# sinamalakouti/CDDMSL

Hardware: AMD Instinct MI355X
Metric: images/sec (train step) VOC+Clipart RN50-C4 (higher is better)
Workload: dtype bf16

## Files before the change

cddmsl_amd/csrc/gemm_conv.hip:

```cpp
#include "common.h"
#include <cstdlib>
#include <type_traits>

namespace {

constexpr int BM = 128, BN = 128, KCH = 8;

struct FastDiv {
  unsigned mul, shr, d;
};
static inline FastDiv make_fastdiv(unsigned d) {
  FastDiv f;
  f.d = d;
  unsigned s = 0;
  while ((1ull << s) < d) ++s;
  f.shr = s;
  f.mul = (unsigned)(((1ull << 32) * ((1ull << s) - d)) / d + 1);
  return f;
}
__device__ __forceinline__ unsigned fdiv(unsigned n, const FastDiv& f) { return (__umulhi(n, f.mul) + n) >> f.shr; }

template <typename T> __device__ __forceinline__ float affine(float v, float sc, float bi) {
  return sizeof(T) <= 2 ? __builtin_fmaf(v, sc, bi) : v * sc + bi;
}
// ... 467 lines not shown
      }
  }

  stage(0);
  for (int kt = 0; kt < nkt; ++kt) {
    const int cur = kt & 1;
    if (kt + 1 < nkt) {
      stage(cur ^ 1);
      asm volatile("s_waitcnt vmcnt(8)" ::: "memory");
    } else {
      asm volatile("s_waitcnt vmcnt(0)" ::: "memory");
    }
    __builtin_amdgcn_s_barrier();
    u32x4 fa[2][2], fb[2][2];
#pragma unroll
    for (int i = 0; i < 2; ++i) {
      fa[0][i] = lds[cur][0][swz(wm * 64 + i * 32 + r, h)];
      fb[0][i] = lds[cur][1][swz(wn * 64 + i * 32 + r, h)];
    }
#pragma unroll
    for (int ks = 0; ks < KCH / 2; ++ks) {
      if (ks + 1 < KCH / 2) {
#pragma unroll
        for (int i = 0; i < 2; ++i) {
          fa[(ks + 1) & 1][i] = lds[cur][0][swz(wm * 64 + i * 32 + r, 2 * (ks + 1) + h)];
          fb[(ks + 1) & 1][i] = lds[cur][1][swz(wn * 64 + i * 32 + r, 2 * (ks + 1) + h)];
        }
      }
#pragma unroll
      for (int a = 0; a < 2; ++a)
#pragma unroll
        for (int b = 0; b < 2; ++b) Mma<T>::step(acc[a][b], fa[ks & 1][a], fb[ks & 1][b]);
    }
    asm volatile("s_waitcnt lgkmcnt(0)" ::: "memory");
    __builtin_amdgcn_s_barrier();
  }

  if (vec_ok) {
    float* ep = (float*)&lds[0][0][0] + wv * 2048;
    const int cg = lane & 7, rr = lane >> 3;
    const int n = n0 + wn * 64 + cg * 8;
    float sc[8], bi[8];
#pragma unroll
    for (int j = 0; j < 8; ++j) {
      sc[j] = (p.scale && n + j < p.Cout) ? p.scale[n + j] : 1.f;
      bi[j] = (p.bias && n + j < p.Cout) ? p.bias[n + j] : 0.f;
    }
#pragma unroll
    for (int a = 0; a < 2; ++a) {
      __syncthreads();
#pragma unroll
      for (int b = 0; b < 2; ++b)
#pragma unroll
        for (int g = 0; g < 16; ++g) {
          int row = (g & 3) + 8 * (g >> 2) + 4 * h, col = b * 32 + r;
          ep[row * 64 + ((((col >> 3) ^ (row & 7)) << 3) | (col & 7))] = acc[a][b][g];
        }
      __syncthreads();
      if (n < p.Cout) {
#pragma unroll
        for (int i = 0; i < 4; ++i) {
          int row = rr + 8 * i;
          int m = m0 + wm * 64 + a * 32 + row;
          if (m >= p.M) continue;
          const f32x4* src = (const f32x4*)(ep + row * 64 + ((cg ^ (row & 7)) << 3));
          f32x4 v0 = src[0], v1 = src[1];
          float v[8] = {v0[0], v0[1], v0[2], v0[3], v1[0], v1[1], v1[2], v1[3]};
#pragma unroll
          for (int j = 0; j < 8; ++j) v[j] = affine<T>(v[j], sc[j], bi[j]);
          if (p.residual) {
            float rv[8];
            if (rf32) load8<float>(p.residual + ((long)m * p.ldr + n) * 4, rv);
            else if (PRE) {
#pragma unroll
              for (int j = 0; j < 4; ++j) { rv[2 * j] = bf2f(rres[a][i][j] & 0xffff); rv[2 * j + 1] = bf2f(rres[a][i][j] >> 16); }
            } else if (p.res_pool) {
              const long po = pooled_row(p, m);
#pragma unroll
              for (int j = 0; j < 8; ++j) rv[j] = 0.f;
              if (po >= 0) load8<T>(p.residual + (po * p.ldr + n) * Mma<T>::ES, rv);
            } else load8<T>(p.residual + ((long)m * p.ldr + n) * Mma<T>::ES, rv);
            if (p.res_pool) {
#pragma unroll
              for (int j = 0; j < 8; ++j) rv[j] *= 0.25f;
            }
#pragma unroll
            for (int j = 0; j < 8; ++j) v[j] += rv[j];
          }
          if (p.relu) {
#pragma unroll
            for (int j = 0; j < 8; ++j) v[j] = fmaxf(v[j], 0.f);
          }
          if (p.relu_mask) {
            float mv[8];
            if (PRE) {
#pragma unroll
              for (int j = 0; j < 4; ++j) { mv[2 * j] = bf2f(rmsk[a][i][j] & 0xffff); mv[2 * j + 1] = bf2f(rmsk[a][i][j] >> 16); }
            } else load8<T>(p.relu_mask + ((long)m * p.ldm + n) * Mma<T>::ES, mv);
#pragma unroll
            for (int j = 0; j < 8; ++j) if (!(mv[j] > 0.f)) v[j] = 0.f;
          }
          if (p.out_f32 || Mma<T>::ES == 4) {
            f32x4* dst = (f32x4*)(p.y + ((long)m * p.ldy + n) * 4);
            f32x4 o0 = {v[0], v[1], v[2], v[3]}, o1 = {v[4], v[5], v[6], v[7]};
            dst[0] = o0; dst[1] = o1;
          } else {
            u32x4 o = {pack2bf(v[0], v[1]), pack2bf(v[2], v[3]), pack2bf(v[4], v[5]), pack2bf(v[6], v[7])};
            *(u32x4*)(p.y + ((long)m * p.ldy + n) * 2) = o;
          }
        }
      }
    }
    return;
  }
#pragma unroll
  for (int b = 0; b < 2; ++b) {
    int n = n0 + wn * 64 + b * 32 + r;
    if (n >= p.Cout) continue;
    float sc = p.scale ? p.scale[n] : 1.f;
    float bi = p.bias ? p.bias[n] : 0.f;
#pragma unroll
    for (int a = 0; a < 2; ++a) {
#pragma unroll
      for (int g = 0; g < 16; ++g) {
        int m = m0 + wm * 64 + a * 32 + (g & 3) + 8 * (g >> 2) + 4 * h;
        if (m >= p.M) continue;
        float v = affine<T>(acc[a][b][g], sc, bi);
        if (p.residual) v += Mma<T>::load(p.residual + ((long)m * p.ldr + n) * Mma<T>::ES);
        if (p.relu) v = fmaxf(v, 0.f);
        if (p.relu_mask && !(Mma<T>::load(p.relu_mask + ((long)m * p.ldm + n) * Mma<T>::ES) > 0.f)) v = 0.f;
        if (p.out_f32) *(float*)(p.y + ((long)m * p.ldy + n) * 4) = v;
        else Mma<T>::store(p.y + ((long)m * p.ldy + n) * Mma<T>::ES, v);
      }
    }
  }
}

struct WgradArgs {
  const char* x;
  const char* dy;
  float* dw;
  const float* scale;
  int Nimg, Hi, Wi, Cin, Ho, Wo, Cout, KH, KW, stride, pad, ldd, pool;
  int M, Kc, cpp, K, ncc;
  int mtiles_per_split;
  FastDiv dWo, dHo;
  int xrs;
  int ldo;
  int direct;
  long bx, bd, bo;
  const float* g0 = nullptr;
  const unsigned long long* mbits = nullptr;
  float* gpos = nullptr;
  float* ws = nullptr;
#ifdef CDDMSL_TILE_STAMPS
  unsigned long long* tstamps = nullptr;
#endif
};

constexpr int WM = 64;
constexpr int WROW = 16 + 4;

template <typename T> struct TrFrag;
template <> struct TrFrag<__bf16> {
  __device__ static __forceinline__ u32x4 read(const u32x4* base, int mrow0, int col0, int lane) {
    int g = lane >> 4, li = lane & 15, q = li >> 2, pp = li & 3;
    int hh = g >> 1;
    int col = col0 + 16 * (g & 1) + 4 * pp;
    const char* b = (const char*)base;
    const char* a0 = b + (long)(mrow0 + 8 * hh + q) * (WROW * 16) + col * 2;
    const char* a1 = a0 + 4 * (WROW * 16);
    i16x4 v0 = __builtin_amdgcn_ds_read_tr16_b64_v4i16((__attribute__((address_space(3))) i16x4*)a0);
    i16x4 v1 = __builtin_amdgcn_ds_read_tr16_b64_v4i16((__attribute__((address_space(3))) i16x4*)a1);
    u32x2 p0 = __builtin_bit_cast(u32x2, v0), p1 = __builtin_bit_cast(u32x2, v1);
    u32x4 r = {p0[0], p0[1], p1[0], p1[1]};
    return r;
  }
  static constexpr int MSTEP = 16;
};
template <> struct TrFrag<float> {
  __device__ static __forceinline__ u32x4 read(const u32x4* base, int mrow0, int col0, int lane) {
    int r = lane & 31, hh = lane >> 5;
    const char* b = (const char*)base;
    u32x4 v;
#pragma unroll
    for (int j = 0; j < 4; ++j) v[j] = *(const unsigned int*)(b + (long)(mrow0 + 4 * hh + j) * (WROW * 16) + (col0 + r) * 4);
    return v;
  }
  static constexpr int MSTEP = 8;
};

template <typename T>
__global__ __launch_bounds__(256, 2) void k_conv_wgrad(WgradArgs p) {
  constexpr int ES = Mma<T>::ES;
  constexpr int TC = 128 * ES / 16;
  constexpr int COLS = 256 / ES;
  __shared__ __attribute__((aligned(16))) u32x4 lds[2][WM * WROW];
  const int t = threadIdx.x, lane = t & 63, wv = t >> 6;
  const int ntn = (p.Cout + COLS - 1) / COLS, ntk = (p.K + COLS - 1) / COLS;
  int bid = xcd_remap(blockIdx.x, gridDim.x);
  const int tile_k = bid % ntk; bid /= ntk;
  const int tile_n = bid % ntn; bid /= ntn;
  const int split = bid;
  const int n0 = tile_n * COLS, k0 = tile_k * COLS;
  const int mt0 = split * p.mtiles_per_split;
  const int total_mt = (p.M + WM - 1) / WM;
  const int mt1 = min(mt0 + p.mtiles_per_split, total_mt);
  (void)TC;

  const int cc = t & 15, rb = t >> 4;
  const int kc = k0 * ES / 16 + cc;
  const bool vk = kc < p.Kc;
  const int pp = vk ? kc / p.cpp : 0, coff = vk ? kc - pp * p.cpp : 0;
  const int ky = pp / p.KW, kx = pp - ky * p.KW;
  const int nc = n0 * ES / 16 + cc;
  const bool vn = nc < p.ncc;
  const u32x4 zero = {0u, 0u, 0u, 0u};
  u32x4 rx[4], rd[4];

  auto gload = [&](int mt) {
#pragma unroll
    for (int i = 0; i < 4; ++i) {
      int m = mt * WM + rb + 16 * i;
      bool vmm = m < p.M;
      unsigned mm = vmm ? m : 0;
      unsigned tq = fdiv(mm, p.dWo);
      int ox = (int)(mm - tq * p.Wo);
      unsigned img = fdiv(tq, p.dHo);
      int oy = (int)(tq - img * p.Ho);
      if (!p.pool) {
        int iy = oy * p.stride - p.pad + ky, ix = ox * p.stride - p.pad + kx;
        bool ok = vmm && vk && iy >= 0 && iy < p.Hi && ix >= 0 && ix < p.Wi;
        rx[i] = ok ? *(const u32x4*)(p.x + ((((long)img * p.Hi + iy) * p.Wi + ix) * p.cpp + coff) * 16) : zero;
      } else {
        if (vmm && vk) {
          const char* b0 = p.x + ((((long)img * p.Hi + 2 * oy) * p.Wi + 2 * ox) * p.cpp + coff) * 16;
          long rs = (long)p.Wi * p.cpp * 16, cs = (long)p.cpp * 16;
          rx[i] = avg4<T>(*(const u32x4*)b0, *(const u32x4*)(b0 + cs), *(const u32x4*)(b0 + rs), *(const u32x4*)(b0 + rs + cs));
        } else rx[i] = zero;
      }
      rd[i] = (vmm && vn) ? *(const u32x4*)(p.dy + ((long)m * p.ldd) * ES + (long)nc * 16) : zero;
    }
  };

  constexpr int WT = COLS / 2;
  constexpr int NT = WT / 32;
  const int wn = wv >> 1, wk = wv & 1;
  f32x16 acc[NT][NT];
#pragma unroll
  for (int a = 0; a < NT; ++a)
#pragma unroll
    for (int b = 0; b < NT; ++b)
#pragma unroll
      for (int r = 0; r < 16; ++r) acc[a][b][r] = 0.f;

  if (mt0 < mt1) gload(mt0);
  for (int mt = mt0; mt < mt1; ++mt) {
#pragma unroll
    for (int i = 0; i < 4; ++i) {
      int row = rb + 16 * i;
      lds[0][row * WROW + cc] = rd[i];
      lds[1][row * WROW + cc] = rx[i];
    }
    __syncthreads();
    if (mt + 1 < mt1) gload(mt + 1);
#pragma unroll
    for (int ms = 0; ms < WM; ms += TrFrag<T>::MSTEP) {
      u32x4 fa[NT], fb[NT];
#pragma unroll
      for (int i = 0; i < NT; ++i) {
        fa[i] = TrFrag<T>::read(lds[0], ms, wn * WT + i * 32, lane);
        fb[i] = TrFrag<T>::read(lds[1], ms, wk * WT + i * 32, lane);
      }
#pragma unroll
      for (int a = 0; a < NT; ++a)
#pragma unroll
        for (int b = 0; b < NT; ++b) Mma<T>::step(acc[a][b], fa[a], fb[b]);
    }
    __syncthreads();
  }

  const int r = lane & 31, h = lane >> 5;
#pragma unroll
  for (int a = 0; a < NT; ++a)
#pragma unroll
    for (int b = 0; b < NT; ++b) {
      int k = k0 + wk * WT + b * 32 + r;
      if (k >= p.K) continue;
#pragma unroll
      for (int g = 0; g < 16; ++g) {
        int n = n0 + wn * WT + a * 32 + (g & 3) + 8 * (g >> 2) + 4 * h;
        if (n >= p.Cout) continue;
        float v = acc[a][b][g] * (p.scale ? p.scale[n] : 1.f);
        atomicAdd(p.dw + (long)n * p.K + k, v);
      }
    }
}

__device__ __forceinline__ int fsw(int row) { return ((row & 3) << 2) | ((row >> 2) & 3); }

template <typename T> struct TrFragS;
template <> struct TrFragS<__bf16> {
  struct Off { int o0, o1; };
  __device__ static __forceinline__ Off prep(int col0, int lane) {
    int g = lane >> 4, li = lane & 15, q = li >> 2, pp = li & 3;
    int hh = g >> 1;
// ... 328 lines not shown
    const char* db = p.dy + (long)(b0 + sb) * p.bd + ac * 16;
    const char* xb = p.x + (long)(b0 + sb) * p.bx + (long)kc * 16;
#pragma unroll
    for (int i = 0; i < 2; ++i) {
      const int m = ar + 32 * i;
      glds16((va && m < p.M) ? db + ((long)m * p.ldd) * 2 : zp, base + (i * 256 + wvu * 64) * 16);
    }
#pragma unroll
    for (int i = 0; i < 4; ++i) {
      const int m = xr + 16 * i;
      glds16((vk && m < p.M) ? xb + ((long)m * p.xrs) * 16 : zp, base + 8192 + (i * 256 + wvu * 64) * 16);
    }
    ++sb;
  };
  f32x16 acc[NTN];
#pragma unroll
  for (int a = 0; a < NTN; ++a)
#pragma unroll
    for (int r = 0; r < 16; ++r) acc[a][r] = 0.f;
  const unsigned lbase = (unsigned)(size_t)(__attribute__((address_space(3))) char*)lds;
  unsigned aoff[NTN][2], xoff[2];
  {
    const int g = lane >> 4, li = lane & 15, q = li >> 2, pp = li & 3, hh = g >> 1;
#pragma unroll
    for (int a = 0; a < NTN; ++a) {
      const int col = a * 32 + 16 * (g & 1) + 4 * pp;
      aoff[a][0] = (8 * hh + q) * 128 + col * 2;
      aoff[a][1] = aoff[a][0] + 4 * 128;
    }
    const TrFragS<__bf16>::Off o = TrFragS<__bf16>::prep(wvu * 32, lane);
    xoff[0] = 8192 + o.o0; xoff[1] = 8192 + o.o1;
  }
  const int r = lane & 31, h = lane >> 5;
  f32x16 gacc[MODE == 3 ? NTN : 1];
  if (MODE == 3) {
#pragma unroll
    for (int a = 0; a < NTN; ++a)
#pragma unroll
      for (int g = 0; g < 16; ++g) gacc[a][g] = 0.f;
  }
  if (nit > 0) stage(0);
  if (nit > 1) stage(1);
  auto item = [&](int it, auto KIND) {
    constexpr int kind = decltype(KIND)::value;
    const int slot = it % NST;
    float g0v = 0.f;
    u32x2 mbv = {~0u, ~0u};
    if (MODE == 3) {
      const long ci = (long)(b0 + it) * p.K + k0 + wvu * 32 + r;
      const char* gp = (const char*)(p.g0 + ci);
      const char* mp = (const char*)(p.mbits + ci);
      asm volatile("global_load_dword %0, %1, off" : "=v"(g0v) : "v"(gp) : "memory");
      asm volatile("global_load_dwordx2 %0, %1, off" : "=v"(mbv) : "v"(mp) : "memory");
    }
    if (kind == 2) {
      stage((it + 2) % NST);
      if (it) wait_vm<12 + NML + NSTORE>(); else wait_vm<12 + NML>();
    } else if (kind == 1) {
      if (it) wait_vm<6 + NML + NSTORE>(); else wait_vm<6 + NML>();
    } else {
      wait_vm<0>();
    }
    __builtin_amdgcn_s_barrier();
    const unsigned sbase = lbase + slot * STAGE;
#define CDDMSL_TRS(DST, A0, A1, IMM)                                                             \
  { u32x2 q0_, q1_;                                                                              \
    asm volatile("ds_read_b64_tr_b16 %0, %1 offset:%2" : "=v"(q0_) : "v"(A0), "i"(IMM));         \
    asm volatile("ds_read_b64_tr_b16 %0, %1 offset:%2" : "=v"(q1_) : "v"(A1), "i"(IMM));         \
    DST = u32x4{q0_[0], q0_[1], q1_[0], q1_[1]}; }
    u32x4 fa[NTN][4], fb[4];
    const unsigned x0 = sbase + xoff[0], x1 = sbase + xoff[1];
    CDDMSL_TRS(fb[0], x0, x1, 0) CDDMSL_TRS(fb[1], x0, x1, 4096) CDDMSL_TRS(fb[2], x0, x1, 8192) CDDMSL_TRS(fb[3], x0, x1, 12288)
#pragma unroll
    for (int a = 0; a < NTN; ++a) {
      const unsigned a0 = sbase + aoff[a][0], a1 = sbase + aoff[a][1];
      CDDMSL_TRS(fa[a][0], a0, a1, 0) CDDMSL_TRS(fa[a][1], a0, a1, 2048) CDDMSL_TRS(fa[a][2], a0, a1, 4096) CDDMSL_TRS(fa[a][3], a0, a1, 6144)
    }
#undef CDDMSL_TRS
    if (NTN == 1) asm volatile("s_waitcnt lgkmcnt(0)" : "+v"(fb[0]), "+v"(fb[1]), "+v"(fb[2]), "+v"(fb[3]), "+v"(fa[0][0]), "+v"(fa[0][1]),
                               "+v"(fa[0][2]), "+v"(fa[0][3]) :: "memory");
    else asm volatile("s_waitcnt lgkmcnt(0)" : "+v"(fb[0]), "+v"(fb[1]), "+v"(fb[2]), "+v"(fb[3]), "+v"(fa[0][0]), "+v"(fa[0][1]), "+v"(fa[0][2]),
                      "+v"(fa[0][3]), "+v"(fa[NTN - 1][0]), "+v"(fa[NTN - 1][1]), "+v"(fa[NTN - 1][2]), "+v"(fa[NTN - 1][3]) :: "memory");
    __builtin_amdgcn_sched_barrier(0);
#pragma unroll
    for (int ms = 0; ms < 4; ++ms)
#pragma unroll
      for (int a = 0; a < NTN; ++a) Mma<__bf16>::step(acc[a], fa[a][ms], fb[ms]);
    __builtin_amdgcn_s_barrier();
    char* outp = (char*)p.dw + (long)(b0 + it) * p.bo;
    const int k = k0 + wvu * 32 + r;
    if (MODE == 3) {
      if (kind == 2) asm volatile("s_waitcnt vmcnt(6)" : "+v"(g0v), "+v"(mbv) :: "memory");
      else asm volatile("s_waitcnt vmcnt(0)" : "+v"(g0v), "+v"(mbv) :: "memory");
      const unsigned a00 = __builtin_bit_cast(unsigned, acc[0][0]);
      const float t0 = __builtin_bit_cast(float, __builtin_amdgcn_permlane32_swap(a00, a00, false, false)[0]) + g0v;
      const float base = t0 * (1.0f / (float)(P > 0 ? P : 1));
      const unsigned mlo = mbv[0], mhi = mbv[1];
#pragma unroll
      for (int a = 0; a < NTN; ++a)
#pragma unroll
        for (int g = 0; g < 16; ++g) {
          const int n0 = a * 32 + (g & 3) + 8 * (g >> 2);
          const bool exists = a * 4 + (g >> 2) < NG;
          const bool lo_ok = n0 >= 1 && n0 <= P, hi_ok = n0 + 4 >= 1 && n0 + 4 <= P;
          if (exists) {
            const int n = n0 + 4 * h;
            const float v = acc[a][g];
            gacc[a][g] += (n == 0) ? t0 : v;
            if (lo_ok || hi_ok) {
              if (h ? hi_ok : lo_ok) {
                const unsigned word = (n - 1) < 32 ? mlo : mhi;
                const bool keep = (word >> ((n - 1) & 31)) & 1u;
                Mma<__bf16>::store(outp + ((long)(n - 1) * p.ldo + k) * 2, keep ? v + base : 0.f);
              }
            }
          }
          acc[a][g] = 0.f;
        }
      return;
    }
#pragma unroll
    for (int a = 0; a < NTN; ++a)
#pragma unroll
      for (int g = 0; g < 16; ++g) {
        if (a * 4 + (g >> 2) < NG) {
          const int n = a * 32 + (g & 3) + 8 * (g >> 2) + 4 * h;
          const float v = acc[a][g];
          const long o = (long)n * p.ldo + k;
          if (MODE == 0) atomicAdd((float*)outp + o, v);
          else if (MODE == 1) ((float*)outp)[o] = v;
          else Mma<__bf16>::store(outp + o * 2, v);
        }
        acc[a][g] = 0.f;
      }
  };
  {
    int it = 0;
    for (; it + 2 < nit; ++it) item(it, std::integral_constant<int, 2>{});
    if (it + 1 < nit) { item(it, std::integral_constant<int, 1>{}); ++it; }
    if (it < nit) item(it, std::integral_constant<int, 0>{});
  }
  if (MODE == 3 && p.gpos) {
    const int k = k0 + wvu * 32 + r;
#pragma unroll
    for (int a = 0; a < NTN; ++a)
#pragma unroll
      for (int g = 0; g < 16; ++g) {
        const int n = a * 32 + (g & 3) + 8 * (g >> 2) + 4 * h;
        if (a * 4 + (g >> 2) < NG && n <= P) atomicAdd(p.gpos + (long)n * p.K + k, gacc[a][g]);
      }
  }
}

__global__ __launch_bounds__(512) void k_wgrad256(WgradArgs p) {
  __shared__ __attribute__((aligned(16))) u32x4 lds[2 * 2 * 2 * 64 * 16];
  const int t = threadIdx.x, lane = t & 63;
#ifdef CDDMSL_TILE_STAMPS
  const unsigned long long ts_entry = __builtin_amdgcn_s_memrealtime();
  unsigned long long ts_loop = ts_entry;
#endif
  p.x += (long)blockIdx.y * p.bx; p.dy += (long)blockIdx.y * p.bd;
  char* outp = (char*)p.dw + (long)blockIdx.y * p.bo;
  const int wvu = __builtin_amdgcn_readfirstlane(t >> 6);
  const int wn = wvu >> 2, wk = wvu & 3;
  const int ntn = p.Cout >> 8, ntk = p.K >> 8;
  int bid = xcd_remap(blockIdx.x, gridDim.x);
  const int tile_k = bid % ntk; bid /= ntk;
  const int tile_n = bid % ntn; bid /= ntn;
  const int n0 = tile_n * 256, k0 = tile_k * 256;
  const int mt0 = bid * p.mtiles_per_split;
  const int nmt = min(p.mtiles_per_split, (p.M + WM - 1) / WM - mt0);
  const bool taps = !(p.KH == 1 && p.KW == 1);

  const int rb = t >> 4, cl = (t & 15) ^ fsw(rb);
  const int gd = (cl >> 3) * 16 + (cl & 7);
  const int gx = (cl >> 2) * 8 + (cl & 3);
  const int kc = (k0 >> 3) + gx;
  const int pp = kc / p.cpp, coff = kc - pp * p.cpp;
  const int ky = pp / p.KW, kx = pp - ky * p.KW;
  unsigned vd[2], vx[2];
#pragma unroll
  for (int i = 0; i < 2; ++i) {
    vd[i] = (unsigned)((i * 32 + rb) * p.ldd * 2 + gd * 16);
    vx[i] = (unsigned)((((i * 32 + rb) + ky * p.Wi + kx) * p.xrs + coff) * 16);
  }
  const __amdgpu_buffer_rsrc_t rd = __builtin_amdgcn_make_buffer_rsrc((void*)(p.dy + ((long)mt0 * WM * p.ldd + n0) * 2), 0, 0x80000000u, 0x00020000);
  const __amdgpu_buffer_rsrc_t rx = __builtin_amdgcn_make_buffer_rsrc((void*)(p.x + ((long)mt0 * WM - p.pad * p.Wi - p.pad) * p.xrs * 16), 0, 0x80000000u, 0x00020000);
  const unsigned dstep = (unsigned)(WM * p.ldd * 2), xstep = (unsigned)(WM * p.xrs * 16);
  const int mrow = mt0 * WM + rb;

  char* const L = (char*)lds;
  auto stageD = [&](auto H, int buf, int T) {
    constexpr int h = decltype(H)::value;
    char* dst = L + (buf << 16) + (h << 14) + wvu * 1024;
#pragma unroll
    for (int i = 0; i < 2; ++i) {
      const unsigned inv = (mrow + T * WM + i * 32 < p.M) ? 0u : 0x80000000u;
      __builtin_amdgcn_raw_ptr_buffer_load_lds(rd, (__attribute__((address_space(3))) void*)(dst + i * 8192 - h * 128), 16,
                                               (int)(vd[i] | inv), (int)(T * dstep), h * 128, 0);
    }
  };
  unsigned xinv[2];
  auto validX = [&](int T) {
#pragma unroll
    for (int i = 0; i < 2; ++i) {
      const int m = mrow + T * WM + i * 32;
      bool ok = m < p.M;
      if (taps) {
        const unsigned mm = min((unsigned)m, (unsigned)(p.M - 1));
        const unsigned tq = fdiv(mm, p.dWo);
        const unsigned ox = mm - tq * p.Wo;
        const unsigned oy = tq - fdiv(tq, p.dHo) * p.Ho;
        ok = ok & ((unsigned)((int)oy - p.pad + ky) < (unsigned)p.Hi) & ((unsigned)((int)ox - p.pad + kx) < (unsigned)p.Wi);
      }
      xinv[i] = ok ? 0u : 0x80000000u;
    }
  };
  auto stageX = [&](auto J, int buf, int T) {
    constexpr int j = decltype(J)::value;
    char* dst = L + (buf << 16) + (1 << 15) + (j << 14) + wvu * 1024;
#pragma unroll
    for (int i = 0; i < 2; ++i)
      __builtin_amdgcn_raw_ptr_buffer_load_lds(rx, (__attribute__((address_space(3))) void*)(dst + i * 8192 - j * 64), 16,
                                               (int)(vx[i] | xinv[i]), (int)(T * xstep), j * 64, 0);
  };
  using I0 = std::integral_constant<int, 0>;
  using I1 = std::integral_constant<int, 1>;

  f32x16 acc[4][2];
#pragma unroll
  for (int a = 0; a < 4; ++a)
#pragma unroll
    for (int b = 0; b < 2; ++b)
#pragma unroll
      for (int r = 0; r < 16; ++r) acc[a][b][r] = 0.f;

  const unsigned lbase = (unsigned)(size_t)(__attribute__((address_space(3))) char*)L;
  unsigned adA[2][2], adB[2];
  {
#pragma unroll
    for (int a = 0; a < 2; ++a) {
      const TrFragS<__bf16>::Off o = TrFragS<__bf16>::prep(wn * 64 + a * 32, lane);
      adA[a][0] = lbase + o.o0; adA[a][1] = lbase + o.o1;
    }
    const TrFragS<__bf16>::Off o = TrFragS<__bf16>::prep(wk * 32, lane);
    adB[0] = lbase + (1u << 15) + o.o0; adB[1] = lbase + (1u << 15) + o.o1;
  }
  u32x4 fa0[2][4], fa1[2][4], fb0[4], fb1[4];
#define CDDMSL_TR2(DST, A0, A1, IMM)                                                             \
  { u32x2 q0_, q1_;                                                                              \
    asm volatile("ds_read_b64_tr_b16 %0, %1 offset:%2" : "=v"(q0_) : "v"(A0), "i"(IMM));         \
    asm volatile("ds_read_b64_tr_b16 %0, %1 offset:%2" : "=v"(q1_) : "v"(A1), "i"(IMM));         \
    DST = u32x4{q0_[0], q0_[1], q1_[0], q1_[1]}; }
#define CDDMSL_READ_A(HALF, FA)                                                                  \
  _Pragma("unroll") for (int a = 0; a < 2; ++a) {                                                \
    CDDMSL_TR2(FA[a][0], adA[a][0], adA[a][1], ((HALF) << 14) + 0 * 4096)                        \
    CDDMSL_TR2(FA[a][1], adA[a][0], adA[a][1], ((HALF) << 14) + 1 * 4096)                        \
    CDDMSL_TR2(FA[a][2], adA[a][0], adA[a][1], ((HALF) << 14) + 2 * 4096)                        \
    CDDMSL_TR2(FA[a][3], adA[a][0], adA[a][1], ((HALF) << 14) + 3 * 4096) }
#define CDDMSL_READ_B(HALF, FB)                                                                  \
  CDDMSL_TR2(FB[0], adB[0], adB[1], ((HALF) << 14) + 0 * 4096)                                   \
  CDDMSL_TR2(FB[1], adB[0], adB[1], ((HALF) << 14) + 1 * 4096)                                   \
  CDDMSL_TR2(FB[2], adB[0], adB[1], ((HALF) << 14) + 2 * 4096)                                   \
  CDDMSL_TR2(FB[3], adB[0], adB[1], ((HALF) << 14) + 3 * 4096)
#define CDDMSL_FLIP_A() { adA[0][0] ^= 1u << 16; adA[0][1] ^= 1u << 16; adA[1][0] ^= 1u << 16; adA[1][1] ^= 1u << 16; }
#define CDDMSL_FLIP_B() { adB[0] ^= 1u << 16; adB[1] ^= 1u << 16; }
#define CDDMSL_MMA_QUAD(I, J, FA, FB)                                               \
  _Pragma("unroll") for (int ms = 0; ms < 4; ++ms) {                                \
    Mma<__bf16>::step(acc[2 * (I)][J], FA[0][ms], FB[ms]);                          \
    Mma<__bf16>::step(acc[2 * (I) + 1][J], FA[1][ms], FB[ms]);                      \
  }
#define CDDMSL_WAIT4(F) asm volatile("s_waitcnt lgkmcnt(0)" : "+v"(F[0]), "+v"(F[1]), "+v"(F[2]), "+v"(F[3]) :: "memory");
#define CDDMSL_WAIT8(F) asm volatile("s_waitcnt lgkmcnt(0)" : "+v"(F[0][0]), "+v"(F[0][1]), "+v"(F[0][2]), "+v"(F[0][3]), \
                                     "+v"(F[1][0]), "+v"(F[1][1]), "+v"(F[1][2]), "+v"(F[1][3]) :: "memory");
#define CDDMSL_PHASE_SYNC_IN(WAIT)                                                  \
  __builtin_amdgcn_sched_barrier(0);                                                \
  __builtin_amdgcn_s_barrier();                                                     \
  WAIT                                                                              \
  __builtin_amdgcn_sched_barrier(0);                                                \
  __builtin_amdgcn_s_setprio(1);
#define CDDMSL_PHASE_SYNC_OUT(I, J)                                                 \
  asm volatile("" : "+v"(acc[2 * (I)][J]), "+v"(acc[2 * (I) + 1][J]));              \
  __builtin_amdgcn_s_setprio(0);                                                    \
  __builtin_amdgcn_sched_barrier(0);                                                \
  __builtin_amdgcn_s_barrier();                                                     \
  __builtin_amdgcn_sched_barrier(0);

  if (nmt > 0) {
    validX(0);
    stageD(I0{}, 0, 0); stageD(I1{}, 0, 0); stageX(I0{}, 0, 0); stageX(I1{}, 0, 0);
    if (nmt > 1) {
      validX(1);
      stageD(I0{}, 1, 1); stageX(I0{}, 1, 1); stageX(I1{}, 1, 1);
      asm volatile("s_waitcnt vmcnt(6)" ::: "memory");
    } else {
      asm volatile("s_waitcnt vmcnt(0)" ::: "memory");
    }
    __builtin_amdgcn_s_barrier();
    __builtin_amdgcn_sched_barrier(0);
    CDDMSL_READ_A(0, fa0)
    CDDMSL_WAIT8(fa0)
    if (wn == 1) __builtin_amdgcn_s_barrier();
    __builtin_amdgcn_sched_barrier(0);
#ifdef CDDMSL_TILE_STAMPS
    ts_loop = __builtin_amdgcn_s_memrealtime();
#endif

    for (int kt = 0; kt < nmt; ++kt) {
      const int d = kt & 1;
      const bool more1 = kt + 1 < nmt, more2 = kt + 2 < nmt;
      CDDMSL_READ_B(0, fb0)
      if (more1) stageD(I1{}, d ^ 1, kt + 1);
      CDDMSL_PHASE_SYNC_IN(CDDMSL_WAIT4(fb0))
      CDDMSL_MMA_QUAD(0, 0, fa0, fb0);
      CDDMSL_PHASE_SYNC_OUT(0, 0)
      CDDMSL_READ_B(1, fb1)
      CDDMSL_FLIP_B()
      if (more2) { stageD(I0{}, d, kt + 2); validX(kt + 2); }
      CDDMSL_PHASE_SYNC_IN(CDDMSL_WAIT4(fb1))
      CDDMSL_MMA_QUAD(0, 1, fa0, fb1);
      CDDMSL_PHASE_SYNC_OUT(0, 1)
      CDDMSL_READ_A(1, fa1)
      CDDMSL_FLIP_A()
      if (more2) {
        stageX(I0{}, d, kt + 2);
        asm volatile("s_waitcnt vmcnt(4)" ::: "memory");
      } else {
        asm volatile("s_waitcnt vmcnt(0)" ::: "memory");
      }
      CDDMSL_PHASE_SYNC_IN(CDDMSL_WAIT8(fa1))
      CDDMSL_MMA_QUAD(1, 1, fa1, fb1);
      CDDMSL_PHASE_SYNC_OUT(1, 1)
      if (more1) { CDDMSL_READ_A(0, fa0) }
      if (more2) stageX(I1{}, d, kt + 2);
      CDDMSL_PHASE_SYNC_IN(CDDMSL_WAIT8(fa0))
      CDDMSL_MMA_QUAD(1, 0, fa1, fb0);
      CDDMSL_PHASE_SYNC_OUT(1, 0)
    }
    if (wn == 0) __builtin_amdgcn_s_barrier();
  }
#undef CDDMSL_TR2
#undef CDDMSL_WAIT4
#undef CDDMSL_WAIT8
#undef CDDMSL_READ_A
#undef CDDMSL_READ_B
#undef CDDMSL_FLIP_A
#undef CDDMSL_FLIP_B
#undef CDDMSL_MMA_QUAD
#undef CDDMSL_PHASE_SYNC_IN
#undef CDDMSL_PHASE_SYNC_OUT

#ifdef CDDMSL_TILE_STAMPS
  const unsigned long long ts_epi = __builtin_amdgcn_s_memrealtime();
#endif
  const int r = lane & 31, h = lane >> 5;
  if (p.ws) {
    f32x4* dst = (f32x4*)p.ws + ((long)(bid * ntn + tile_n) * ntk + tile_k) * (8 * 32 * 64) + (wvu * 32) * 64 + lane;
#pragma unroll
    for (int a = 0; a < 4; ++a)
#pragma unroll
      for (int b = 0; b < 2; ++b)
#pragma unroll
        for (int g4 = 0; g4 < 4; ++g4) {
          const f32x4 v = {acc[a][b][4 * g4], acc[a][b][4 * g4 + 1], acc[a][b][4 * g4 + 2], acc[a][b][4 * g4 + 3]};
          dst[((a * 2 + b) * 4 + g4) * 64] = v;
        }
  } else
#pragma unroll
  for (int a = 0; a < 4; ++a)
#pragma unroll
    for (int b = 0; b < 2; ++b) {
      const int k = k0 + wk * 64 + b * 32 + r;
#pragma unroll
// ... 218 lines not shown
        if (wf) Mma<T>::store(wf + i * ES, v);
        if (scale) v *= scale[co];
      }
      tile[ty + 8 * r][tx] = v;
    }
    __syncthreads();
    if (wd) {
#pragma unroll
      for (int r = 0; r < 4; ++r) {
        const int ci = it * 32 + ty + 8 * r, co = ct * 32 + tx;
        if (ci < Cin && co < Cout) {
          const long j = (((long)ci * KH + (KH - 1 - ky)) * KW + (KW - 1 - kx)) * Cout + co;
          Mma<T>::store(wd + j * ES, tile[tx][ty + 8 * r]);
        }
      }
    }
  }
}
template <typename T>
__global__ __launch_bounds__(256) void k_weight_prep(const float* w, const float* scale, char* wf, char* wd, int Cout, int KH, int KW, int Cin) {
  weight_prep_body<T>(w, scale, wf, wd, Cout, KH, KW, Cin, (long)blockIdx.x, (long)gridDim.x);
}
template <typename T>
__global__ __launch_bounds__(256) void k_weight_prep_multi(const long long* table) {
  const long long* e = table + 8 * (long)blockIdx.y;
  weight_prep_body<T>((const float*)e[0], (const float*)e[1], (char*)e[2], (char*)e[3], (int)e[4], (int)e[5], (int)e[6], (int)e[7],
                      (long)blockIdx.x, (long)gridDim.x);
}

template <typename T, int CPP, int NT, int NTAP = 9>
__global__ __launch_bounds__(256) void k_conv3x3_small(ConvArgs p) {
  constexpr int KC = NTAP * CPP, KS = (KC + 1) / 2;
  constexpr int PAD = NTAP == 9 ? 1 : 0;
  constexpr int ES = Mma<T>::ES;
  const int lane = threadIdx.x & 63, r = lane & 31, hh = lane >> 5;
  constexpr bool WLDS = CPP > 1;
  __shared__ __attribute__((aligned(16))) u32x4 wl[WLDS ? NT * KS * 64 : 1];
  u32x4 bw[WLDS ? 1 : NT][WLDS ? 1 : KS];
  {
    const int wv = threadIdx.x >> 6;
#pragma unroll
    for (int nt = 0; nt < NT; ++nt)
#pragma unroll
      for (int ks = 0; ks < KS; ++ks) {
        if (WLDS && ((nt * KS + ks) & 3) != wv) continue;
        const int q = 2 * ks + hh;
        u32x4 v = {0u, 0u, 0u, 0u};
        if (q < KC) v = *(const u32x4*)(p.w + ((long)(nt * 32 + r) * KC + q) * 16);
        if (WLDS) wl[(nt * KS + ks) * 64 + lane] = v;
        else bw[WLDS ? 0 : nt][WLDS ? 0 : ks] = v;
      }
    if (WLDS) __syncthreads();
  }
  float sc[NT], bi[NT];
#pragma unroll
  for (int nt = 0; nt < NT; ++nt) { sc[nt] = p.scale ? p.scale[nt * 32 + r] : 1.f; bi[nt] = p.bias ? p.bias[nt * 32 + r] : 0.f; }
  const int wave = (blockIdx.x * blockDim.x + threadIdx.x) >> 6, nwaves = (gridDim.x * blockDim.x) >> 6;
  const int ntiles = (p.M + 31) >> 5;
  const __amdgpu_buffer_rsrc_t rx = __builtin_amdgcn_make_buffer_rsrc((void*)(p.x - (long)(p.Wi + 1) * (CPP * 16)), 0, 0x7fffffff, 0x00020000);
  const long ybytes = (long)p.M * p.ldy * ES, mbytes = (long)p.M * p.ldm * ES;
  const __amdgpu_buffer_rsrc_t ry = __builtin_amdgcn_make_buffer_rsrc((void*)p.y, 0, (int)(ybytes > 0x7fffffffL ? 0x7fffffffL : ybytes), 0x00020000);
  const __amdgpu_buffer_rsrc_t rm = __builtin_amdgcn_make_buffer_rsrc((void*)p.relu_mask, 0, p.relu_mask ? (int)(mbytes > 0x7fffffffL ? 0x7fffffffL : mbytes) : 0, 0x00020000);
  const float relu_floor = p.relu ? 0.f : -__builtin_inff();
  __shared__ __attribute__((aligned(16))) u32x4 ost[ES == 2 ? 4 * 32 * NT * 4 : 1];
  const bool ost_ok = !p.relu_mask && p.ldy == NT * 32 && (long)p.M * NT * 64 < 0x7fffffffL;
  for (int tile = wave; tile < ntiles; tile += nwaves) {
    const int m = tile * 32 + r;
    const bool vm = m < p.M;
    const unsigned mm = vm ? m : 0;
    const unsigned tq = fdiv(mm, p.dWo), ox = mm - tq * p.Wo;
    const unsigned img = fdiv(tq, p.dHo), oy = tq - img * p.Ho;
    const int iy0 = (int)oy * p.stride - PAD, ix0 = (int)ox * p.stride - PAD;
    const unsigned lbase = (unsigned)((((int)img * p.Hi + iy0 + 1) * p.Wi + ix0 + 1) * (CPP * 16)) + (CPP > 1 ? hh * 16 : 0);
    unsigned bad = vm ? 0u : 0x1ffu;
    if (NTAP == 9) {
#pragma unroll
      for (int ky = 0; ky < 3; ++ky)
#pragma unroll
        for (int kx = 0; kx < 3; ++kx)
          if ((unsigned)(iy0 + ky) >= (unsigned)p.Hi || (unsigned)(ix0 + kx) >= (unsigned)p.Wi) bad |= 1u << (3 * ky + kx);
    }
    u32x4 a[KS];
#pragma unroll
    for (int ks = 0; ks < KS; ++ks) {
      const int q0 = 2 * ks, q1 = 2 * ks + 1;
      const int t0 = q0 / CPP, c0 = q0 % CPP, t1 = q1 / CPP, c1 = q1 % CPP;
      if (CPP > 1) {
        const unsigned v = lbase | (__builtin_amdgcn_ubfe(bad, (unsigned)t0, 1u) << 31);
        a[ks] = __builtin_amdgcn_raw_buffer_load_b128(rx, v, ((t0 / 3) * p.Wi + (t0 % 3)) * (CPP * 16) + c0 * 16, 0);
      } else {
        const int ky = hh ? t1 / 3 : t0 / 3, kx = hh ? t1 % 3 : t0 % 3, cc = hh ? c1 : c0;
        const bool inq = hh ? (q1 < KC) : (q0 < KC);
        const int iy = iy0 + ky, ix = ix0 + kx;
        const bool ok = vm && inq && (unsigned)iy < (unsigned)p.Hi && (unsigned)ix < (unsigned)p.Wi;
        u32x4 v = {0u, 0u, 0u, 0u};
        if (ok) v = *(const u32x4*)(p.x + ((((long)img * p.Hi + iy0) * p.Wi + ix0) + (long)ky * p.Wi + kx) * (CPP * 16) + cc * 16);
        a[ks] = v;
      }
    }
    f32x16 acc[NT];
#pragma unroll
    for (int nt = 0; nt < NT; ++nt)
#pragma unroll
      for (int g = 0; g < 16; ++g) acc[nt][g] = 0.f;
    int wlane = lane;
    asm volatile("" : "+v"(wlane));
#pragma unroll
    for (int ks = 0; ks < KS; ++ks)
#pragma unroll
      for (int nt = 0; nt < NT; ++nt) {
        if (WLDS) Mma<T>::step(acc[nt], a[ks], wl[(nt * KS + ks) * 64 + wlane]);
        else Mma<T>::step(acc[nt], a[ks], bw[WLDS ? 0 : nt][WLDS ? 0 : ks]);
      }
    if (ES == 2 && ost_ok) {
      char* ob = (char*)ost + (threadIdx.x >> 6) * (32 * NT * 64);
#pragma unroll
      for (int nt = 0; nt < NT; ++nt)
#pragma unroll
        for (int g = 0; g < 16; ++g) {
          const int row = (g & 3) + 8 * (g >> 2) + 4 * hh;
          float v = affine<T>(acc[nt][g], sc[nt], bi[nt]);
          asm("v_max_f32 %0, %1, %2" : "=v"(v) : "v"(v), "s"(relu_floor));
          *(unsigned short*)(ob + row * (NT * 64) + (nt * 32 + r) * 2) = f2bf(v);
        }
#pragma unroll
      for (int i = 0; i < 2 * NT; ++i) {
        const u32x4 o = *(const u32x4*)(ob + (i * 64 + lane) * 16);
        __builtin_amdgcn_raw_buffer_store_b128(o, ry, (unsigned)((i * 64 + lane) * 16), tile * (32 * NT * 64), 0);
      }
      continue;
    }
    const unsigned vy = (unsigned)(((tile * 32 + 4 * hh) * p.ldy + r) * ES), vmk = (unsigned)(((tile * 32 + 4 * hh) * p.ldm + r) * ES);
#pragma unroll
    for (int nt = 0; nt < NT; ++nt)
#pragma unroll
      for (int g = 0; g < 16; ++g) {
        const int row = (g & 3) + 8 * (g >> 2);
        float v = affine<T>(acc[nt][g], sc[nt], bi[nt]);
        asm("v_max_f32 %0, %1, %2" : "=v"(v) : "v"(v), "s"(relu_floor));
        if (p.relu_mask) {
          float mv;
          if (ES == 2) mv = bf2f((unsigned)__builtin_amdgcn_raw_buffer_load_b16(rm, vmk, (row * p.ldm + nt * 32) * ES, 0));
          else mv = __builtin_bit_cast(float, __builtin_amdgcn_raw_buffer_load_b32(rm, vmk, (row * p.ldm + nt * 32) * ES, 0));
          if (!(mv > 0.f)) v = 0.f;
        }
        if (ES == 2) __builtin_amdgcn_raw_buffer_store_b16((unsigned short)f2bf(v), ry, vy, (row * p.ldy + nt * 32) * ES, 0);
        else __builtin_amdgcn_raw_buffer_store_b32(__builtin_bit_cast(unsigned, v), ry, vy, (row * p.ldy + nt * 32) * ES, 0);
      }
  }
}

static thread_local int g_last_kernel = 0;
static thread_local int g_plan_only = 0;
static thread_local int g_batch = 1;
static inline int g_batch_peek() { return g_batch; }

__device__ __forceinline__ void blds16(__amdgpu_buffer_rsrc_t r, unsigned voff, unsigned soff, void* l) {
  __builtin_amdgcn_raw_ptr_buffer_load_lds(r, (__attribute__((address_space(3))) void*)l, 16, (int)voff, (int)soff, 0, 0);
}

template <typename T, bool RPOOL, int EPI, bool PRE = false>
__device__ __forceinline__ void tile_epilogue(const ConvArgs& p, f32x16 (&acc)[4][2], float* ep, int wr, int wc, int lane, int m0, int n0,
                                              const u32x4 (*pre)[4] = nullptr, const f32x4* sb = nullptr) {
  constexpr int ES = Mma<T>::ES;
  const int r32 = lane & 31, hh = lane >> 5;
  const int cg = lane & 7, rr = lane >> 3;
  const int n = n0 + wc * 64 + cg * 8;
  float sc[8], bi[8];
#pragma unroll
  for (int j = 0; j < 8; ++j) {
    if (sb) { sc[j] = sb[j >> 2][j & 3]; bi[j] = sb[2 + (j >> 2)][j & 3]; }
    else { sc[j] = p.scale ? p.scale[n + j] : 1.f; bi[j] = p.bias ? p.bias[n + j] : 0.f; }
  }
  const bool has_res = EPI < 0 ? p.residual != nullptr : (EPI & 1) != 0;
  const bool has_msk = EPI < 0 ? p.relu_mask != nullptr : (EPI & 2) != 0;
  const bool f32out = EPI < 0 && (ES == 4 || p.out_f32 != 0);
  const int eso = f32out ? 4 : 2;
  const float relu_floor = p.relu ? 0.f : -__builtin_inff();
  const long rows = p.M - m0;
  auto mk = [&](const char* base, long ld, int es) {
    long bytes = rows * ld * es;
    if (bytes > 0x7fffffffL) bytes = 0x7fffffffL;
    return __builtin_amdgcn_make_buffer_rsrc((void*)(base + (long)m0 * ld * es), 0, base ? (int)bytes : 0, 0x00020000);
  };
  const bool rf32 = EPI < 0 && ES == 2 && p.res_f32;
  const int esr = rf32 ? 4 : ES;
  const __amdgpu_buffer_rsrc_t ry = mk(p.y, p.ldy, eso), rmsk = mk(p.relu_mask, p.ldm, ES);
  const __amdgpu_buffer_rsrc_t rres = RPOOL ? __builtin_amdgcn_make_buffer_rsrc((void*)p.residual, 0, 0x7fffffff, 0x00020000)
                                            : mk(p.residual, p.ldr, esr);
  auto pooled_off = [&](int m) -> unsigned {
    const unsigned tq = fdiv((unsigned)m, p.dWo), ox = m - tq * p.Wo;
    const unsigned img = fdiv(tq, p.dHo), oy = tq - img * p.Ho;
    const unsigned hp = p.Ho >> 1, wp = p.Wo >> 1;
    const bool in = m < p.M && (oy >> 1) < hp && (ox >> 1) < wp;
    return in ? (unsigned)((((img * hp + (oy >> 1)) * wp + (ox >> 1)) * (unsigned)p.ldr + (unsigned)n) * ES) : 0x80000000u;
  };
  const unsigned vy = (unsigned)(((wr * 128 + rr) * p.ldy + n) * eso);
  const unsigned vr = (unsigned)(((wr * 128 + rr) * p.ldr + n) * esr), vm = (unsigned)(((wr * 128 + rr) * p.ldm + n) * ES);
  const bool emit8 = EPI < 0 && ES == 2 && p.y8 != nullptr;
  const __amdgpu_buffer_rsrc_t ry8 = mk(p.y8, p.ldy, 1);
  const unsigned vy8 = (unsigned)((wr * 128 + rr) * p.ldy + n);
  const float q8s = emit8 && p.q8 ? p.q8[0] : 1.f;
  unsigned am8 = 0u;
  constexpr int DEPTH = ES == 2 ? 2 : 1;
  char* wbase[8];
#pragma unroll
  for (int c = 0; c < 8; ++c)
    wbase[c] = (char*)ep + (hh * 4 * 64 + ((((r32 >> 3) ^ (hh << 2)) ^ c) << 3) + (r32 & 7)) * 4;
  u32x4 rresb[DEPTH][4][ES / 2], rmskb[DEPTH][4][ES / 2];
  auto fetch = [&](int a, u32x4 (*rres_)[ES / 2], u32x4 (*rmsk_)[ES / 2]) {
#pragma unroll
    for (int i = 0; i < 4; ++i)
#pragma unroll
      for (int q = 0; q < ES / 2; ++q) {
        if (RPOOL) rres_[i][q] = __builtin_amdgcn_raw_buffer_load_b128(rres, pooled_off(m0 + wr * 128 + a * 32 + rr + 8 * i), q * 16, 0);
        else if (has_res && !rf32) rres_[i][q] = __builtin_amdgcn_raw_buffer_load_b128(rres, vr, (a * 32 + 8 * i) * p.ldr * ES + q * 16, CDDMSL_LOAD_AUX);
        if (has_msk) rmsk_[i][q] = __builtin_amdgcn_raw_buffer_load_b128(rmsk, vm, (a * 32 + 8 * i) * p.ldm * ES + q * 16, CDDMSL_LOAD_AUX);
      }
  };
  if (PRE && DEPTH == 2) {
#pragma unroll
    for (int d = 0; d < 2; ++d)
#pragma unroll
      for (int i = 0; i < 4; ++i) {
        if (EPI & 1) {
          rresb[d % DEPTH][i][0] = pre[d][i];
          if (EPI & 2) rmskb[d % DEPTH][i][0] = __builtin_amdgcn_raw_buffer_load_b128(rmsk, vm, (d * 32 + 8 * i) * p.ldm * ES, CDDMSL_LOAD_AUX);
        } else rmskb[d % DEPTH][i][0] = pre[d][i];
      }
  } else if (DEPTH == 2 && !rf32) { fetch(0, rresb[0], rmskb[0]); fetch(1, rresb[DEPTH - 1], rmskb[DEPTH - 1]); }
  auto put = [&](auto A) {
    constexpr int a = decltype(A)::value;
#pragma unroll
    for (int b = 0; b < 2; ++b)
#pragma unroll
      for (int g = 0; g < 16; ++g)
        *(float*)(wbase[(b << 2) ^ (g & 3)] + ((g & 3) + 8 * (g >> 2)) * 256 + (a & 1) * 8192) = acc[a][b][g];
  };
  auto pass = [&](auto A) {
    constexpr int a = decltype(A)::value;
    if (DEPTH == 1) fetch(a, rresb[0], rmskb[0]);
    if (rf32) {
#pragma unroll
      for (int f = 0; f < 8; ++f)
        rresb[(f >> 2) % DEPTH][f & 3][0] = __builtin_amdgcn_raw_buffer_load_b128(rres, vr, (a * 32 + 8 * (f >> 1)) * p.ldr * 4 + (f & 1) * 16, 0);
    }
    u32x4 (*rres_)[ES / 2] = rresb[a % DEPTH];
    u32x4 (*rmsk_)[ES / 2] = rmskb[a % DEPTH];
    asm volatile("s_waitcnt lgkmcnt(0)" ::: "memory");
    f32x4 val[4][2];
#pragma unroll
    for (int i = 0; i < 4; ++i) {
      const int row = rr + 8 * i;
      const f32x4* src = (const f32x4*)(ep + (a & 1) * 2048 + row * 64 + ((cg ^ (row & 7)) << 3));
      val[i][0] = src[0]; val[i][1] = src[1];
    }
    asm volatile("" ::: "memory");
    if constexpr (a + 1 < 4) put(std::integral_constant<int, a + 1>{});
    asm volatile("" ::: "memory");
#pragma unroll
    for (int i = 0; i < 4; ++i) {
      const f32x4 v0 = val[i][0], v1 = val[i][1];
      float v[8] = {v0[0], v0[1], v0[2], v0[3], v1[0], v1[1], v1[2], v1[3]};
#pragma unroll
      for (int j = 0; j < 8; ++j) v[j] = affine<T>(v[j], sc[j], bi[j]);
      if (rf32) {
#pragma unroll
        for (int j = 0; j < 4; ++j) {
          v[j] += __builtin_bit_cast(f32x4, rresb[((2 * i) >> 2) % DEPTH][(2 * i) & 3][0])[j];
          v[4 + j] += __builtin_bit_cast(f32x4, rresb[((2 * i + 1) >> 2) % DEPTH][(2 * i + 1) & 3][0])[j];
        }
      } else if (RPOOL) {
        if (ES == 2) {
#pragma unroll
          for (int j = 0; j < 4; ++j) { v[2 * j] += 0.25f * bf2f(rres_[i][0][j] & 0xffff); v[2 * j + 1] += 0.25f * bf2f(rres_[i][0][j] >> 16); }
        } else {
#pragma unroll
          for (int j = 0; j < 4; ++j) {
            v[j] += 0.25f * __builtin_bit_cast(f32x4, rres_[i][0])[j]; v[4 + j] += 0.25f * __builtin_bit_cast(f32x4, rres_[i][ES / 2 - 1])[j];
          }
        }
      } else if (has_res) {
        if (ES == 2) {
#pragma unroll
          for (int j = 0; j < 4; ++j) { v[2 * j] += bf2f(rres_[i][0][j] & 0xffff); v[2 * j + 1] += bf2f(rres_[i][0][j] >> 16); }
        } else {
#pragma unroll
          for (int j = 0; j < 4; ++j) {
            v[j] += __builtin_bit_cast(f32x4, rres_[i][0])[j]; v[4 + j] += __builtin_bit_cast(f32x4, rres_[i][ES / 2 - 1])[j];
          }
        }
      }
#pragma unroll
      for (int j = 0; j < 8; ++j) asm("v_max_f32 %0, %1, %2" : "=v"(v[j]) : "v"(v[j]), "s"(relu_floor));
      if (has_msk) {
        float mv[8];
        if (ES == 2) {
#pragma unroll
          for (int j = 0; j < 4; ++j) { mv[2 * j] = bf2f(rmsk_[i][0][j] & 0xffff); mv[2 * j + 1] = bf2f(rmsk_[i][0][j] >> 16); }
        } else {
#pragma unroll
          for (int j = 0; j < 4; ++j) {
            mv[j] = __builtin_bit_cast(f32x4, rmsk_[i][0])[j]; mv[4 + j] = __builtin_bit_cast(f32x4, rmsk_[i][ES / 2 - 1])[j];
          }
        }
#pragma unroll
        for (int j = 0; j < 8; ++j) if (!(mv[j] > 0.f)) v[j] = 0.f;
      }
      const unsigned so = (unsigned)((a * 32 + 8 * i) * p.ldy * eso);
      if (emit8) {
#pragma unroll
        for (int j = 0; j < 8; ++j) am8 = absmax_bits(am8, v[j]);
        const u32x2 o8 = {pack4_e4m3(v[0] * q8s, v[1] * q8s, v[2] * q8s, v[3] * q8s), pack4_e4m3(v[4] * q8s, v[5] * q8s, v[6] * q8s, v[7] * q8s)};
        __builtin_amdgcn_raw_buffer_store_b64(o8, ry8, vy8, (unsigned)((a * 32 + 8 * i) * p.ldy), CDDMSL_STORE_AUX);
        asm volatile("s_nop 4" ::: "memory");
        asm volatile("" :: "v"(o8));
      }
      if (f32out) {
        const u32x4 o0 = {__builtin_bit_cast(unsigned, v[0]), __builtin_bit_cast(unsigned, v[1]), __builtin_bit_cast(unsigned, v[2]), __builtin_bit_cast(unsigned, v[3])};
        const u32x4 o1 = {__builtin_bit_cast(unsigned, v[4]), __builtin_bit_cast(unsigned, v[5]), __builtin_bit_cast(unsigned, v[6]), __builtin_bit_cast(unsigned, v[7])};
        __builtin_amdgcn_raw_buffer_store_b128(o0, ry, vy, so, CDDMSL_STORE_AUX);
        __builtin_amdgcn_raw_buffer_store_b128(o1, ry, vy, so + 16, CDDMSL_STORE_AUX);
        asm volatile("s_nop 4" ::: "memory");
        asm volatile("" :: "v"(o0), "v"(o1));
      } else {
        const u32x4 o = {pack2bf(v[0], v[1]), pack2bf(v[2], v[3]), pack2bf(v[4], v[5]), pack2bf(v[6], v[7])};
        if (p.nt_out) __builtin_amdgcn_raw_buffer_store_b128(o, ry, vy, so, CDDMSL_STORE_AUX);
        else __builtin_amdgcn_raw_buffer_store_b128(o, ry, vy, so, 0);
        asm volatile("s_nop 4" ::: "memory");
        asm volatile("" :: "v"(o));
      }
    }
    if (DEPTH == 2 && a + 2 < 4 && !rf32) fetch(a + 2, rresb[a % DEPTH], rmskb[a % DEPTH]);
  };
  put(std::integral_constant<int, 0>{});
  pass(std::integral_constant<int, 0>{});
  pass(std::integral_constant<int, 1>{});
  pass(std::integral_constant<int, 2>{});
  pass(std::integral_constant<int, 3>{});
  if (emit8 && p.amax8) {
    am8 = wave_max_u(am8);
    if (lane == 0) atomicMax(p.amax8 + (blockIdx.x & 63), am8);
  }
}

template <typename T, bool TAPS, bool RPOOL = false, int EPI = -1, bool PERSIST = false, bool SPLITK = false>
__global__ __launch_bounds__(512) void k_conv_fwd256(ConvArgs p) {
  __shared__ __attribute__((aligned(16))) u32x4 lds[2 * 2 * 2 * 128 * KCH];
  const int t_in = threadIdx.x;
  p.x += (long)blockIdx.y * p.bx; p.w += (long)blockIdx.y * p.bw; p.y += (long)blockIdx.y * p.by;
  const int ntn = p.Cout >> 8;
  const int ntiles = PERSIST ? (p.tile_limit ? p.tile_limit : ntn * ((p.M + 255) >> 8)) : 0;
  int lbid = PERSIST ? (int)((blockIdx.x & 7) * (gridDim.x >> 3) + (blockIdx.x >> 3))
           : SPLITK ? p.tile0 + (int)(blockIdx.x / (unsigned)p.ksplits) : xcd_remap(blockIdx.x, gridDim.x);
  const int kt0 = SPLITK ? (int)(blockIdx.x % (unsigned)p.ksplits) * p.kper : 0;
  if (PERSIST && lbid >= ntiles) return;
  for (;;) {
  int t = t_in;
  if (PERSIST) asm volatile("" : "+v"(t));
  const int lane = t & 63;
#ifdef CDDMSL_TILE_STAMPS
  const unsigned long long ts_entry = __builtin_amdgcn_s_memrealtime();
#endif
  const int wvu = __builtin_amdgcn_readfirstlane(t >> 6);
  const int wr = wvu >> 2, wc = wvu & 3;
  const int tile_n = lbid % ntn, tile_m = lbid / ntn;
  const int m0 = tile_m * 256, n0 = tile_n * 256;
  const int cl = (t & 7) ^ ((t >> 4) & 7);
  const int nkt = SPLITK ? min(p.kper, (p.Kc >> 3) - kt0) : (p.Kc >> 3);
  const int tpt = p.cpp >> 3;

  auto rowoff = [&](int m, int& iy0, int& ix0) {
    const unsigned tq = fdiv((unsigned)m, p.dWo), ox = m - tq * p.Wo;
    const unsigned img = fdiv(tq, p.dHo), oy = tq - img * p.Ho;
    iy0 = (int)oy * p.stride - p.pad; ix0 = (int)ox * p.stride - p.pad;
    return (((long)img * p.Hi + iy0) * p.Wi + ix0) * p.xrs * 16;
  };
  int iyb, ixb;
  const long base_a = rowoff(m0, iyb, ixb);
  const __amdgpu_buffer_rsrc_t ra_rsrc = __builtin_amdgcn_make_buffer_rsrc((void*)(p.x + base_a), 0, 0x7fffffff, 0x00020000);
  const __amdgpu_buffer_rsrc_t rb_rsrc = __builtin_amdgcn_make_buffer_rsrc((void*)(p.w + (long)n0 * p.wrs * 16), 0, 0x7fffffff, 0x00020000);
  unsigned va[2][2], vinv[2][2], vb[2][2];
  int iy0[2][2], ix0[2][2];
#pragma unroll
  for (int h = 0; h < 2; ++h)
#pragma unroll
    for (int i = 0; i < 2; ++i) {
      const int m = m0 + i * 128 + h * 64 + (t >> 3);
      const bool vm = m < p.M;
      const long ro = rowoff(vm ? m : m0, iy0[h][i], ix0[h][i]);
      va[h][i] = (unsigned)(ro - base_a) + cl * 16;
      if (!vm) { iy0[h][i] = -(1 << 20); if (!TAPS) va[h][i] |= 0x80000000u; }
      vinv[h][i] = 0;
      vb[h][i] = (unsigned)(((2 * i + (t >> 8)) * 64 + h * 32 + ((t >> 3) & 31)) * p.wrs + cl) * 16;
    }
  if (TAPS) {
    unsigned xm[2][2] = {{0, 0}, {0, 0}};
    for (int kx = 0; kx < p.KW; ++kx)
#pragma unroll
      for (int h = 0; h < 2; ++h)
#pragma unroll
        for (int i = 0; i < 2; ++i) xm[h][i] |= ((unsigned)(ix0[h][i] + kx) >= (unsigned)p.Wi ? 1u : 0u) << kx;
    const unsigned full = (1u << p.KW) - 1u;
    for (int ky = 0; ky < p.KH; ++ky)
#pragma unroll
      for (int h = 0; h < 2; ++h)
#pragma unroll
        for (int i = 0; i < 2; ++i) vinv[h][i] |= ((unsigned)(iy0[h][i] + ky) >= (unsigned)p.Hi ? full : xm[h][i]) << (ky * p.KW);
  }
  const int step_col = (p.xrs - (p.cpp - KCH)) * 16;
  const int step_row = ((p.Wi - (p.KW - 1)) * p.xrs - (p.cpp - KCH)) * 16;
  int left[2] = {tpt, tpt}, tap[2] = {0, 0}, kxs[2] = {0, 0};
  unsigned soa[2] = {0, 0}, sob[2] = {0, 0};
  if (SPLITK) {
    const int tap0 = TAPS ? kt0 / tpt : 0, within = TAPS ? kt0 - tap0 * tpt : kt0;
    const int ky0 = TAPS ? tap0 / p.KW : 0, kx0 = tap0 - ky0 * p.KW;
#pragma unroll
    for (int h = 0; h < 2; ++h) {
      left[h] = tpt - (TAPS ? within : 0); tap[h] = tap0; kxs[h] = kx0;
      soa[h] = (unsigned)((ky0 * p.Wi + kx0) * p.xrs * 16 + within * KCH * 16);
      sob[h] = (unsigned)(kt0 * KCH * 16);
    }
  }

  char* const L = (char*)lds;
  auto stageA = [&](auto H, int buf) {
    constexpr int h = decltype(H)::value;
    char* dst = L + (buf << 16) + (h << 14) + wvu * 1024;
#pragma unroll
    for (int i = 0; i < 2; ++i) {
      unsigned v = va[h][i];
      if (TAPS) v |= __builtin_amdgcn_ubfe(vinv[h][i], (unsigned)tap[h], 1u) << 31;
      blds16(ra_rsrc, v, soa[h], dst + i * 8192);
    }
    if (TAPS) {
      int step = KCH * 16;
      if (--left[h] == 0) {
        left[h] = tpt; ++tap[h];
        if (++kxs[h] == p.KW) { kxs[h] = 0; step = step_row; } else step = step_col;
      }
      soa[h] += step;
    } else soa[h] += KCH * 16;
  };
  auto stageB = [&](auto J, int buf) {
    constexpr int j = decltype(J)::value;
    char* dst = L + (buf << 16) + (1 << 15) + (j << 14) + wvu * 1024;
#pragma unroll
    for (int i = 0; i < 2; ++i) blds16(rb_rsrc, vb[j][i], sob[j], dst + i * 8192);
    sob[j] += KCH * 16;
  };
  using I0 = std::integral_constant<int, 0>;
  using I1 = std::integral_constant<int, 1>;

  f32x16 acc[4][2];
#pragma unroll
  for (int a = 0; a < 4; ++a)
#pragma unroll
    for (int b = 0; b < 2; ++b)
#pragma unroll
      for (int r = 0; r < 16; ++r) acc[a][b][r] = 0.f;

  const int r32 = lane & 31, hh = lane >> 5, sw = (r32 >> 1) & 7;
  unsigned ada[4], adb[4];
#pragma unroll
  for (int ks = 0; ks < 4; ++ks) {
    ada[ks] = (unsigned)(((wr * 64 + r32) * KCH + ((2 * ks + hh) ^ sw)) * 16);
    adb[ks] = (unsigned)(((wc * 32 + r32) * KCH + ((2 * ks + hh) ^ sw)) * 16 + (1 << 15));
  }
  u32x4 fa0[2][4], fa1[2][4], fb0[4], fb1[4];
  auto readA = [&](auto I, u32x4 (*fa)[4]) {
    constexpr int i = decltype(I)::value;
#pragma unroll
    for (int rt = 0; rt < 2; ++rt)
#pragma unroll
      for (int ks = 0; ks < 4; ++ks) fa[rt][ks] = *(const u32x4*)(L + ada[ks] + ((i << 14) + rt * 32 * KCH * 16));
  };
  auto readB = [&](auto J, u32x4* fb) {
    constexpr int j = decltype(J)::value;
#pragma unroll
    for (int ks = 0; ks < 4; ++ks) fb[ks] = *(const u32x4*)(L + adb[ks] + (j << 14));
  };
  auto flipA = [&]() {
#pragma unroll
    for (int ks = 0; ks < 4; ++ks) ada[ks] ^= 1u << 16;
  };
  auto flipB = [&]() {
#pragma unroll
    for (int ks = 0; ks < 4; ++ks) adb[ks] ^= 1u << 16;
  };
#define CDDMSL_MMA_QUAD(I, J, FA, FB) MmaQuad<T>::run(acc[2 * (I)][J], acc[2 * (I) + 1][J], FA, FB)
#ifdef CDDMSL_STAMPS
  unsigned long long st_sum[4] = {0, 0, 0, 0}, st_last = 0;
#define CDDMSL_STAMP(K) { asm volatile("s_waitcnt lgkmcnt(0)" ::: "memory"); unsigned long long tt_ = __builtin_readcyclecounter(); \
                          asm volatile("s_waitcnt lgkmcnt(0)" ::: "memory"); st_sum[K] += tt_ - st_last; st_last = tt_; }
#else
#define CDDMSL_STAMP(K)
#endif
#define CDDMSL_PHASE_SYNC_IN()                                                      \
  CDDMSL_STAMP(0)                                                                   \
  __builtin_amdgcn_sched_barrier(0);                                                \
  __builtin_amdgcn_s_barrier();                                                     \
  asm volatile("s_waitcnt lgkmcnt(0)" ::: "memory");                                \
  CDDMSL_STAMP(1)                                                                   \
  __builtin_amdgcn_sched_barrier(0);                                                \
  __builtin_amdgcn_s_setprio(1);
#define CDDMSL_PHASE_SYNC_OUT(I, J)                                                 \
  asm volatile("" : "+v"(acc[2 * (I)][J]), "+v"(acc[2 * (I) + 1][J]));    \
  __builtin_amdgcn_s_setprio(0);                                                    \
  CDDMSL_STAMP(2)                                                                   \
  __builtin_amdgcn_sched_barrier(0);                                                \
  __builtin_amdgcn_s_barrier();                                                     \
  CDDMSL_STAMP(3)                                                                   \
  __builtin_amdgcn_sched_barrier(0);

  stageA(I0{}, 0); stageA(I1{}, 0); stageB(I0{}, 0); stageB(I1{}, 0);
  if (nkt > 1) {
    stageA(I0{}, 1); stageB(I0{}, 1); stageB(I1{}, 1);
    asm volatile("s_waitcnt vmcnt(6)" ::: "memory");
  } else {
    asm volatile("s_waitcnt vmcnt(0)" ::: "memory");
  }
  __builtin_amdgcn_s_barrier();
  readA(I0{}, fa0);
  if (wr == 1) __builtin_amdgcn_s_barrier();
  __builtin_amdgcn_sched_barrier(0);
#ifdef CDDMSL_STAMPS
  st_last = __builtin_readcyclecounter();
#endif
#ifdef CDDMSL_TILE_STAMPS
  const unsigned long long ts_loop = __builtin_amdgcn_s_memrealtime();
#endif

  constexpr bool PREF = EPI > 0 && !RPOOL && Mma<T>::ES == 2 && !SPLITK;
  u32x4 pre[2][4];
  f32x4 sb[4];
  auto ktile = [&](int kt, auto LAST) {
    constexpr bool last = decltype(LAST)::value;
    const int d = kt & 1;
    const bool more1 = !last, more2 = !last && kt + 2 < nkt;
    readB(I0{}, fb0);
    if (more1) stageA(I1{}, d ^ 1);
    CDDMSL_PHASE_SYNC_IN();
    CDDMSL_MMA_QUAD(0, 0, fa0, fb0);
    CDDMSL_PHASE_SYNC_OUT(0, 0);
    readB(I1{}, fb1);
    flipB();
    if (more2) stageA(I0{}, d);
    CDDMSL_PHASE_SYNC_IN();
    CDDMSL_MMA_QUAD(0, 1, fa0, fb1);
    CDDMSL_PHASE_SYNC_OUT(0, 1);
    readA(I1{}, fa1);
    flipA();
    if (more2) {
      stageB(I0{}, d);
      asm volatile("s_waitcnt vmcnt(4)" ::: "memory");
    } else if (more1) {
      asm volatile("s_waitcnt vmcnt(0)" ::: "memory");
    } else if (PREF) {
      const bool is_res = (EPI & 1) != 0;
      const char* base = is_res ? p.residual : p.relu_mask;
      const int ld = is_res ? p.ldr : p.ldm;
      long bytes = ((long)p.M - m0) * ld * 2;
      if (bytes > 0x7fffffffL) bytes = 0x7fffffffL;
      const __amdgpu_buffer_rsrc_t rs = __builtin_amdgcn_make_buffer_rsrc((void*)(base + (long)m0 * ld * 2), 0, (int)bytes, 0x00020000);
      const unsigned vo = (unsigned)(((wr * 128 + (lane >> 3)) * ld + n0 + wc * 64 + (lane & 7) * 8) * 2);
#pragma unroll
      for (int a = 0; a < 2; ++a)
#pragma unroll
        for (int i = 0; i < 4; ++i) pre[a][i] = __builtin_amdgcn_raw_buffer_load_b128(rs, vo, (a * 32 + 8 * i) * ld * 2, 0);
    }
    CDDMSL_PHASE_SYNC_IN();
    CDDMSL_MMA_QUAD(1, 1, fa1, fb1);
    CDDMSL_PHASE_SYNC_OUT(1, 1);
    if (more1) readA(I0{}, fa0);
    if (more2) stageB(I1{}, d);
    if (last && !SPLITK) {
      const int n = n0 + wc * 64 + (lane & 7) * 8;
      const f32x4 one = {1.f, 1.f, 1.f, 1.f}, zero = {0.f, 0.f, 0.f, 0.f};
      sb[0] = p.scale ? *(const f32x4*)(p.scale + n) : one; sb[1] = p.scale ? *(const f32x4*)(p.scale + n + 4) : one;
      sb[2] = p.bias ? *(const f32x4*)(p.bias + n) : zero; sb[3] = p.bias ? *(const f32x4*)(p.bias + n + 4) : zero;
    }
    CDDMSL_PHASE_SYNC_IN();
    CDDMSL_MMA_QUAD(1, 0, fa1, fb0);
    CDDMSL_PHASE_SYNC_OUT(1, 0);
  };
  for (int kt = 0; kt + 1 < nkt; ++kt) ktile(kt, std::false_type{});
  ktile(nkt - 1, std::true_type{});
  if (wr == 0) __builtin_amdgcn_s_barrier();
#ifdef CDDMSL_TILE_STAMPS
  const unsigned long long ts_epi = __builtin_amdgcn_s_memrealtime();
#endif
#ifdef CDDMSL_STAMPS
  if (p.stamps && lane == 0) {
#pragma unroll
    for (int k = 0; k < 4; ++k) p.stamps[((long)blockIdx.x * 8 + wvu) * 4 + k] = st_sum[k];
  }
#endif
#undef CDDMSL_MMA_QUAD
#undef CDDMSL_PHASE_SYNC_IN
#undef CDDMSL_PHASE_SYNC_OUT
#undef CDDMSL_STAMP

  if (SPLITK) {
    f32x4* dst = (f32x4*)p.partial + (long)blockIdx.x * (8 * 32 * 64) + (wvu * 32) * 64 + lane;
#pragma unroll
    for (int a = 0; a < 4; ++a)
#pragma unroll
      for (int b = 0; b < 2; ++b)
#pragma unroll
        for (int g4 = 0; g4 < 4; ++g4) {
          const f32x4 v = {acc[a][b][4 * g4], acc[a][b][4 * g4 + 1], acc[a][b][4 * g4 + 2], acc[a][b][4 * g4 + 3]};
          dst[((a * 2 + b) * 4 + g4) * 64] = v;
        }
    return;
  }
  tile_epilogue<T, RPOOL, EPI, PREF>(p, acc, (float*)lds + wvu * 4096, wr, wc, lane, m0, n0, pre, sb);
#ifdef CDDMSL_TILE_STAMPS
  if (p.tstamps && lane == 0) {
    if (!PERSIST) asm volatile("s_waitcnt vmcnt(0)" ::: "memory");
    unsigned long long* o = p.tstamps + ((long)(PERSIST ? lbid : (int)blockIdx.x) * 8 + wvu) * 4;
    o[0] = ts_entry; o[1] = ts_loop; o[2] = ts_epi; o[3] = __builtin_amdgcn_s_memrealtime();
  }
#endif
  if (!PERSIST) break;
  lbid += gridDim.x;
  if (lbid >= ntiles) break;
  __builtin_amdgcn_s_barrier();
  }
}

template <typename T, bool TAPS, int EPI>
__global__ __launch_bounds__(256, 2) void k_conv_fwd2(ConvArgs p) {
  constexpr int SA = 256 * 64, SB = 128 * 64, SS = SA + SB, STAGES = 3;
  __shared__ __attribute__((aligned(16))) u32x4 lds[STAGES * SS / 16];
  const int t = threadIdx.x, lane = t & 63;
#ifdef CDDMSL_TILE_STAMPS
  const unsigned long long ts_entry = __builtin_amdgcn_s_memrealtime();
#endif
  p.x += (long)blockIdx.y * p.bx; p.w += (long)blockIdx.y * p.bw; p.y += (long)blockIdx.y * p.by;
  const int wvu = __builtin_amdgcn_readfirstlane(t >> 6);
  const int wr = wvu >> 1, wc = wvu & 1;
  const int ntn = p.Cout >> 7;
  const int lbid = xcd_remap(blockIdx.x, gridDim.x);
  const int tile_n = lbid % ntn, tile_m = lbid / ntn;
  const int m0 = tile_m * 256, n0 = tile_n * 128;
  const int cl = (t & 3) ^ ((t >> 3) & 3);
  const int nkt = p.Kc >> 2;
  const int tpt = p.cpp >> 2;

  auto rowoff = [&](int m, int& iy0, int& ix0) {
    const unsigned tq = fdiv((unsigned)m, p.dWo), ox = m - tq * p.Wo;
    const unsigned img = fdiv(tq, p.dHo), oy = tq - img * p.Ho;
    iy0 = (int)oy * p.stride - p.pad; ix0 = (int)ox * p.stride - p.pad;
    return (((long)img * p.Hi + iy0) * p.Wi + ix0) * p.xrs * 16;
  };
  int iyb, ixb;
  const long base_a = rowoff(m0, iyb, ixb);
  const __amdgpu_buffer_rsrc_t ra_rsrc = __builtin_amdgcn_make_buffer_rsrc((void*)(p.x + base_a), 0, 0x7fffffff, 0x00020000);
  const __amdgpu_buffer_rsrc_t rb_rsrc = __builtin_amdgcn_make_buffer_rsrc((void*)(p.w + (long)n0 * p.wrs * 16), 0, 0x7fffffff, 0x00020000);
  unsigned va[4], vinv[4], vb[2];
  int iy0[4], ix0[4];
#pragma unroll
  for (int i = 0; i < 4; ++i) {
    const int m = m0 + (t >> 2) + 64 * i;
    const bool vm = m < p.M;
    const long ro = rowoff(vm ? m : m0, iy0[i], ix0[i]);
    va[i] = (unsigned)(ro - base_a) + cl * 16;
    if (!vm) { iy0[i] = -(1 << 20); if (!TAPS) va[i] |= 0x80000000u; }
    vinv[i] = 0;
  }
#pragma unroll
  for (int i = 0; i < 2; ++i) vb[i] = (unsigned)((((t >> 2) + 64 * i) * p.wrs + cl) * 16);
  if (TAPS) {
    unsigned xm[4] = {0, 0, 0, 0};
    for (int kx = 0; kx < p.KW; ++kx)
#pragma unroll
      for (int i = 0; i < 4; ++i) xm[i] |= ((unsigned)(ix0[i] + kx) >= (unsigned)p.Wi ? 1u : 0u) << kx;
    const unsigned full = (1u << p.KW) - 1u;
    for (int ky = 0; ky < p.KH; ++ky)
#pragma unroll
      for (int i = 0; i < 4; ++i) vinv[i] |= ((unsigned)(iy0[i] + ky) >= (unsigned)p.Hi ? full : xm[i]) << (ky * p.KW);
  }
  const int step_col = (p.xrs - (p.cpp - 4)) * 16;
  const int step_row = ((p.Wi - (p.KW - 1)) * p.xrs - (p.cpp - 4)) * 16;
  int left = tpt, tap = 0, kxs = 0;
  unsigned soa = 0, sob = 0;

  char* const L = (char*)lds;
  auto stage = [&](int st) {
    char* dst = L + st * SS + wvu * 1024;
#pragma unroll
    for (int i = 0; i < 4; ++i) {
      unsigned v = va[i];
      if (TAPS) v |= __builtin_amdgcn_ubfe(vinv[i], (unsigned)tap, 1u) << 31;
      blds16(ra_rsrc, v, soa, dst + i * 4096);
    }
#pragma unroll
    for (int i = 0; i < 2; ++i) blds16(rb_rsrc, vb[i], sob, dst + SA + i * 4096);
    sob += 64;
    if (TAPS) {
      int step = 64;
      if (--left == 0) {
        left = tpt; ++tap;
        if (++kxs == p.KW) { kxs = 0; step = step_row; } else step = step_col;
      }
      soa += step;
    } else soa += 64;
  };

  f32x16 acc[4][2];
#pragma unroll
  for (int a = 0; a < 4; ++a)
#pragma unroll
    for (int b = 0; b < 2; ++b)
#pragma unroll
      for (int r = 0; r < 16; ++r) acc[a][b][r] = 0.f;

  const int r32 = lane & 31, hh = lane >> 5, sw = (r32 >> 1) & 3;
  unsigned ada[2], adb[2];
#pragma unroll
  for (int ks = 0; ks < 2; ++ks) {
    ada[ks] = (unsigned)(((wr * 128 + r32) * 4 + ((2 * ks + hh) ^ sw)) * 16);
    adb[ks] = (unsigned)(SA + ((wc * 64 + r32) * 4 + ((2 * ks + hh) ^ sw)) * 16);
  }
  u32x4 fa[2][4][2], fb[2][2][2];
  auto readf = [&](auto SET, int st) {
    constexpr int set = decltype(SET)::value;
    const char* base = L + st * SS;
#pragma unroll
    for (int rt = 0; rt < 4; ++rt)
#pragma unroll
      for (int ks = 0; ks < 2; ++ks) fa[set][rt][ks] = *(const u32x4*)(base + ada[ks] + rt * 32 * 64);
#pragma unroll
    for (int ct = 0; ct < 2; ++ct)
#pragma unroll
      for (int ks = 0; ks < 2; ++ks) fb[set][ct][ks] = *(const u32x4*)(base + adb[ks] + ct * 32 * 64);
  };
  using S0 = std::integral_constant<int, 0>;
  using S1 = std::integral_constant<int, 1>;

  stage(0);
  if (nkt > 1) stage(1);
  if (nkt > 2) stage(2);
  if (nkt > 2) asm volatile("s_waitcnt vmcnt(12)" ::: "memory");
  else if (nkt > 1) asm volatile("s_waitcnt vmcnt(6)" ::: "memory");
  else asm volatile("s_waitcnt vmcnt(0)" ::: "memory");
  __builtin_amdgcn_s_barrier();
  readf(S0{}, 0);
#ifdef CDDMSL_TILE_STAMPS
  const unsigned long long ts_loop = __builtin_amdgcn_s_memrealtime();
#endif
  int st_next = 1, st_free = 0;

  auto ktile = [&](int kt, auto SET) {
    constexpr int set = decltype(SET)::value;
    if (kt + 2 < nkt) asm volatile("s_waitcnt vmcnt(6)" ::: "memory");
    else asm volatile("s_waitcnt vmcnt(0)" ::: "memory");
    __builtin_amdgcn_s_waitcnt(0xc07f);
    __builtin_amdgcn_sched_barrier(0);
    __builtin_amdgcn_s_barrier();
    __builtin_amdgcn_sched_barrier(0);
    if (kt + 1 < nkt) readf(std::integral_constant<int, set ^ 1>{}, st_next);
    if (kt + 3 < nkt) stage(st_free);
    st_next = st_next == STAGES - 1 ? 0 : st_next + 1;
    st_free = st_free == STAGES - 1 ? 0 : st_free + 1;
    __builtin_amdgcn_sched_barrier(0);
    __builtin_amdgcn_s_setprio(1);
#pragma unroll
    for (int ks = 0; ks < 2; ++ks)
// ... 12 lines not shown
  asm volatile("" : "+v"(acc[3][1]));
  const unsigned long long ts_epi = __builtin_amdgcn_s_memrealtime();
#endif
  tile_epilogue<T, false, EPI>(p, acc, (float*)lds + wvu * 4096, wr, wc, lane, m0, n0);
#ifdef CDDMSL_TILE_STAMPS
  if (p.tstamps && lane == 0) {
    asm volatile("s_waitcnt vmcnt(0)" ::: "memory");
    unsigned long long* o = p.tstamps + ((long)blockIdx.x * 4 + wvu) * 4;
    o[0] = ts_entry; o[1] = ts_loop; o[2] = ts_epi; o[3] = __builtin_amdgcn_s_memrealtime();
  }
#endif
}

static bool gemm256_legal(const ConvArgs& a) {
  const bool vec_ok = (a.ldy % 8 == 0) && (!a.residual || a.ldr % 8 == 0) && (!a.relu_mask || a.ldm % 8 == 0);
  if (a.pool || (a.cpp & 7) || (a.Cout & 255) || !vec_ok || a.KH * a.KW > 31) return false;
  if (2 * a.pad > a.KH - 1 || 2 * a.pad > a.KW - 1) return false;
  return true;
}
static bool use_gemm256(const ConvArgs& a) {
  const char* e = getenv("CDDMSL_GEMM256");
  const int mode = e ? atoi(e) : 1;
  if (mode == 0) return false;
  if (!gemm256_legal(a)) return false;
  if (mode == 2) return true;
  const long tiles = (long)((a.M + 255) / 256) * (a.Cout / 256) * g_batch_peek();
  return tiles >= 160;
}


__global__ __launch_bounds__(256) void k_conv_split_reduce(ConvArgs p) {
  const int tile_rel = blockIdx.x >> 6, q = (blockIdx.x & 63) * 256 + threadIdx.x;
  const f32x4* src = (const f32x4*)p.partial + (long)tile_rel * p.ksplits * 16384 + q;
  f32x4 sum = src[0];
  for (int s = 1; s < p.ksplits; ++s) sum += src[(long)s * 16384];
  const int wvu = q >> 11, j = (q >> 6) & 31, lane = q & 63, r32 = lane & 31, hh = lane >> 5;
  const int a = j >> 3, b = (j >> 2) & 1, g4 = j & 3, wr = wvu >> 2, wc = wvu & 3;
  const int ntn = p.Cout >> 8, lbid = p.tile0 + tile_rel;
  const int tile_n = lbid % ntn, tile_m = lbid / ntn;
  const int n = tile_n * 256 + wc * 64 + b * 32 + r32;
  const int mrow = tile_m * 256 + wr * 128 + a * 32 + 8 * g4 + 4 * hh;
  const float sc = p.scale ? p.scale[n] : 1.f, bi = p.bias ? p.bias[n] : 0.f;
#pragma unroll
  for (int e = 0; e < 4; ++e) {
    const long m = mrow + e;
    if (m >= p.M) break;
    float v = __builtin_fmaf(sum[e], sc, bi);
    if (p.residual) v += bf2f(*(const unsigned short*)(p.residual + (m * p.ldr + n) * 2));
    if (p.relu) v = fmaxf(v, 0.f);
    if (p.relu_mask && !(bf2f(*(const unsigned short*)(p.relu_mask + (m * p.ldm + n) * 2)) > 0.f)) v = 0.f;
    *(unsigned short*)(p.y + (m * p.ldy + n) * 2) = f2bf(v);
  }
}

static void* g_ws = nullptr;
static long g_ws_bytes = 0;

static int persistent_blocks_raw() {
  static int ncu = -1;
  if (ncu < 0) {
    int dev = 0, n = 0;
    if (hipGetDevice(&dev) != hipSuccess || hipDeviceGetAttribute(&n, hipDeviceAttributeMultiprocessorCount, dev) != hipSuccess) n = 0;
    ncu = (n / 8) * 8;
  }
  return ncu;
}
static int persistent_blocks() {
  const char* e = getenv("CDDMSL_PERSIST");
  return (e ? atoi(e) : 1) ? persistent_blocks_raw() : 0;
}

static bool fwd2_legal(const ConvArgs& a) {
  const bool vec_ok = (a.ldy % 8 == 0) && (!a.residual || a.ldr % 8 == 0) && (!a.relu_mask || a.ldm % 8 == 0);
  if (a.pool || a.res_pool || (a.cpp & 3) || (a.Cout & 127) || !vec_ok || a.KH * a.KW > 31) return false;
  if (2 * a.pad > a.KH - 1 || 2 * a.pad > a.KW - 1) return false;
  return true;
}
static bool use_fwd2(const ConvArgs& a) {
  const char* e = getenv("CDDMSL_FWD2");
  const int mode = e ? atoi(e) : 1;
  if (mode == 0 || !fwd2_legal(a)) return false;
  if (mode == 2) return true;
  if (use_gemm256(a) || g_batch_peek() != 1) return false;
  const char* et = getenv("CDDMSL_FWD2_MIN");
  return (long)(a.Cout / 128) * ((a.M + 255) / 256) >= (et ? atol(et) : 256);
}
template <typename T> void launch_fwd2(const ConvArgs& a, dim3 grid, hipStream_t st) {
  const bool taps = !(a.KH == 1 && a.KW == 1 && a.pad == 0);
  if (sizeof(T) == 4 || a.out_f32 || a.res_f32 || a.y8) {
    if (taps) hipLaunchKernelGGL((k_conv_fwd2<T, true, -1>), grid, dim3(256), 0, st, a);
    else hipLaunchKernelGGL((k_conv_fwd2<T, false, -1>), grid, dim3(256), 0, st, a);
    return;
  }
  if constexpr (sizeof(T) == 2) {
    const int epi = (a.residual ? 1 : 0) | (a.relu_mask ? 2 : 0);
#define CDDMSL_L2(TP, E) hipLaunchKernelGGL((k_conv_fwd2<T, TP, E>), grid, dim3(256), 0, st, a)
    if (taps) { switch (epi) { case 0: CDDMSL_L2(true, 0); break; case 1: CDDMSL_L2(true, 1); break; case 2: CDDMSL_L2(true, 2); break; default: CDDMSL_L2(true, 3); } }
    else { switch (epi) { case 0: CDDMSL_L2(false, 0); break; case 1: CDDMSL_L2(false, 1); break; case 2: CDDMSL_L2(false, 2); break; default: CDDMSL_L2(false, 3); } }
#undef CDDMSL_L2
  }
}

template <typename T, bool TAPS> void launch256_main(const ConvArgs& a, dim3 grid, hipStream_t st, int epi);
constexpr int TAIL_FRAC_DEFAULT = 8;
template <typename T, bool TAPS> void launch256(const ConvArgs& a, dim3 grid, hipStream_t st) {
  if (sizeof(T) == 4 || a.out_f32 || a.res_f32 || a.y8) { hipLaunchKernelGGL((k_conv_fwd256<T, TAPS, false, -1>), grid, dim3(512), 0, st, a); return; }
  const int epi = (a.residual ? 1 : 0) | (a.relu_mask ? 2 : 0);
  if constexpr (std::is_same<T, __bf16>::value) {
    const int ncu = persistent_blocks_raw();
    const int tiles = (int)grid.x, rem = ncu > 0 ? tiles % ncu : 0, nktot = a.Kc >> 3;
    const char* et = getenv("CDDMSL_TAIL_SPLIT");
    const char* ef = getenv("CDDMSL_TAIL_FRAC");
    const int frac = ef ? (atoi(ef) > 0 ? atoi(ef) : 8) : TAIL_FRAC_DEFAULT;
    if (!(et && atoi(et) == 0) && grid.y == 1 && tiles > ncu && rem > 0 && rem * frac <= ncu && nktot >= 16 && g_ws) {
      int S = ncu / rem;
      if (S > nktot / 2) S = nktot / 2;
      { const char* es = getenv("CDDMSL_TAIL_MAXS"); if (es && S > atoi(es)) S = atoi(es); }
      const int kper = (nktot + S - 1) / S;
      S = (nktot + kper - 1) / kper;
      if (S >= 2 && (long)rem * S * 65536 * 4 <= g_ws_bytes) {
        ConvArgs m = a, t = a;
        m.tile_limit = tiles - rem;
        launch256_main<T, TAPS>(m, dim3((unsigned)(tiles - rem), 1), st, epi);
        t.partial = (float*)g_ws; t.tile0 = tiles - rem; t.ksplits = S; t.kper = kper;
        hipLaunchKernelGGL((k_conv_fwd256<T, TAPS, false, -1, false, true>), dim3((unsigned)(rem * S)), dim3(512), 0, st, t);
        hipLaunchKernelGGL(k_conv_split_reduce, dim3((unsigned)(rem * 64)), dim3(256), 0, st, t);
        return;
      }
    }
  }
  launch256_main<T, TAPS>(a, grid, st, epi);
}
template <typename T, bool TAPS> void launch256_main(const ConvArgs& a, dim3 grid, hipStream_t st, int epi) {
  if constexpr (std::is_same<T, __bf16>::value && !TAPS) {
    const int nb = persistent_blocks();
    const char* emk = getenv("CDDMSL_PERSIST_MAXKT");
    if (nb > 0 && grid.y == 1 && (int)grid.x > nb && (a.Kc >> 3) <= (emk ? atoi(emk) : 8)) {
      switch (epi) {
        case 0: hipLaunchKernelGGL((k_conv_fwd256<T, false, false, 0, true>), dim3(nb), dim3(512), 0, st, a); break;
        case 1: hipLaunchKernelGGL((k_conv_fwd256<T, false, false, 1, true>), dim3(nb), dim3(512), 0, st, a); break;
        case 2: hipLaunchKernelGGL((k_conv_fwd256<T, false, false, 2, true>), dim3(nb), dim3(512), 0, st, a); break;
        default: hipLaunchKernelGGL((k_conv_fwd256<T, false, false, 3, true>), dim3(nb), dim3(512), 0, st, a); break;
      }
      return;
    }
  }
  switch (epi) {
    case 0: hipLaunchKernelGGL((k_conv_fwd256<T, TAPS, false, 0>), grid, dim3(512), 0, st, a); break;
    case 1: hipLaunchKernelGGL((k_conv_fwd256<T, TAPS, false, 1>), grid, dim3(512), 0, st, a); break;
    case 2: hipLaunchKernelGGL((k_conv_fwd256<T, TAPS, false, 2>), grid, dim3(512), 0, st, a); break;
    default: hipLaunchKernelGGL((k_conv_fwd256<T, TAPS, false, 3>), grid, dim3(512), 0, st, a); break;
  }
}
template <> void launch256<float, false>(const ConvArgs& a, dim3 grid, hipStream_t st) { hipLaunchKernelGGL((k_conv_fwd256<float, false, false, -1>), grid, dim3(512), 0, st, a); }
template <> void launch256<float, true>(const ConvArgs& a, dim3 grid, hipStream_t st) { hipLaunchKernelGGL((k_conv_fwd256<float, true, false, -1>), grid, dim3(512), 0, st, a); }

template <typename T> int conv_fwd_launch(ConvArgs& a, hipStream_t st) {
  int ntn = (a.Cout + BN - 1) / BN, ntm = (a.M + BM - 1) / BM;
  long grid = (long)ntn * ntm;
  if (grid <= 0) return CDDMSL_OK;
  if (grid > 0x7fffffffL) return CDDMSL_ERR_ARG;
  if (!a.pool && a.KH == 3 && a.KW == 3 && a.pad == 1 && (a.cpp == 1 || a.cpp == 4 || (a.cpp == 8 && a.Cout == 64)) &&
      (a.Cout == 32 || a.Cout == 64) && !a.residual && !a.out_f32 && g_batch == 1 && a.xrs == a.cpp && a.wrs == a.Kc) {
    g_last_kernel = 8;
    if (g_plan_only) return CDDMSL_OK;
    const int nb = a.cpp > 1 ? 256 * 2 : 256 * 8;
    if (a.cpp == 1 && a.Cout == 32) hipLaunchKernelGGL((k_conv3x3_small<T, 1, 1>), dim3(nb), dim3(256), 0, st, a);
    else if (a.cpp == 1) hipLaunchKernelGGL((k_conv3x3_small<T, 1, 2>), dim3(nb), dim3(256), 0, st, a);
    else if (a.cpp == 8) hipLaunchKernelGGL((k_conv3x3_small<T, 8, 2>), dim3(nb), dim3(256), 0, st, a);
    else if (a.Cout == 32) hipLaunchKernelGGL((k_conv3x3_small<T, 4, 1>), dim3(nb), dim3(256), 0, st, a);
    else hipLaunchKernelGGL((k_conv3x3_small<T, 4, 2>), dim3(nb), dim3(256), 0, st, a);
    return launch_status();
  }
  if (sizeof(T) == 2 && !a.pool && a.KH == 1 && a.KW == 1 && a.pad == 0 && a.stride == 1 && a.Cout == 64 && (a.cpp == 8 || a.cpp == 32) &&
      !a.residual && !a.out_f32 && !a.y8 && g_batch == 1 && a.xrs == a.cpp && a.wrs == a.Kc && a.ldy == 64 &&
      !(getenv("CDDMSL_SMALL_1X1") && atoi(getenv("CDDMSL_SMALL_1X1")) == 0)) {
    g_last_kernel = 8;
    if (g_plan_only) return CDDMSL_OK;
    if (a.cpp == 8) hipLaunchKernelGGL((k_conv3x3_small<T, 8, 2, 1>), dim3(512), dim3(256), 0, st, a);
    else hipLaunchKernelGGL((k_conv3x3_small<T, 32, 2, 1>), dim3(512), dim3(256), 0, st, a);
    return launch_status();
  }
  if (use_fwd2(a)) {
    grid = (long)(a.Cout / 128) * ((a.M + 255) / 256);
    g_last_kernel = 11;
    if (g_plan_only) return CDDMSL_OK;
    launch_fwd2<T>(a, dim3((unsigned)grid, (unsigned)g_batch), st);
    return launch_status();
  }
  if (use_gemm256(a)) {
    grid = (long)(a.Cout / 256) * ((a.M + 255) / 256);
    g_last_kernel = 3;
    if (g_plan_only) return CDDMSL_OK;
    const dim3 g256((unsigned)grid, (unsigned)g_batch);
    if (a.res_pool) hipLaunchKernelGGL((k_conv_fwd256<T, false, true>), g256, dim3(512), 0, st, a);
    else if (a.KH == 1 && a.KW == 1 && a.pad == 0) launch256<T, false>(a, g256, st);
    else launch256<T, true>(a, g256, st);
  } else if (a.pool) { g_last_kernel = 2; if (g_plan_only) return CDDMSL_OK; hipLaunchKernelGGL(k_conv_fwd_reg<T>, dim3((unsigned)grid), dim3(256), 0, st, a); }
  else { g_last_kernel = 1; if (g_plan_only) return CDDMSL_OK; hipLaunchKernelGGL(k_conv_fwd<T>, dim3((unsigned)grid, (unsigned)g_batch), dim3(256), 0, st, a); }
  return launch_status();
}

}

#ifdef CDDMSL_TILE_STAMPS
static unsigned long long* g_tile_stamps = nullptr;
extern "C" void cddmsl_debug_tile_stamps(unsigned long long* p) { g_tile_stamps = p; }
#endif
extern "C" int cddmsl_last_kernel(void) { return g_last_kernel; }
extern "C" int cddmsl_plan_only(int on) { const int was = g_plan_only; g_plan_only = on; return was; }

static int nt_out_for(long out_bytes) {
  static const long nt_min_mb = getenv("CDDMSL_NT_MIN_MB") ? atol(getenv("CDDMSL_NT_MIN_MB")) : 128;
  return out_bytes > (nt_min_mb << 20) ? 1 : 0;
}

static int conv_fwd_impl(const void* x, const void* w, void* y, const float* scale, const float* bias,
                         const void* residual, const void* relu_mask, int Nimg, int Hi, int Wi, int Cin,
                         int Cout, int KH, int KW, int stride, int pad, int pool, int ldy, int ldr, int ldm,
                         int relu, int out_f32, int dtype, void* y8, const float* q8, float* amax8, void* stream) {
  int es = dtype == 0 ? 2 : 4;
  if (dtype != 0 && dtype != 1) return CDDMSL_ERR_ARG;
  if (Nimg < 0 || Hi <= 0 || Wi <= 0 || Cin <= 0 || Cout <= 0 || KH <= 0 || KW <= 0 || stride <= 0) return CDDMSL_ERR_ARG;
  if ((Cin * es) % 16 != 0) return CDDMSL_ERR_ARG;
  if (pool && (KH != 1 || KW != 1 || pad != 0 || stride != 1)) return CDDMSL_ERR_ARG;
  ConvArgs a;
  a.x = (const char*)x; a.w = (const char*)w; a.y = (char*)y; a.scale = scale; a.bias = bias;
  a.residual = (const char*)residual; a.relu_mask = (const char*)relu_mask;
  a.Nimg = Nimg; a.Hi = Hi; a.Wi = Wi; a.Cin = Cin; a.Cout = Cout; a.KH = KH; a.KW = KW; a.stride = stride; a.pad = pad;
  if (pool) { a.Ho = Hi / 2; a.Wo = Wi / 2; }
  else { a.Ho = (Hi + 2 * pad - KH) / stride + 1; a.Wo = (Wi + 2 * pad - KW) / stride + 1; }
  if (a.Ho <= 0 || a.Wo <= 0) return CDDMSL_ERR_ARG;
  if ((out_f32 & 2) && (!(out_f32 & 1) || !residual || relu_mask || pool)) return CDDMSL_ERR_ARG;
  a.ldy = ldy; a.ldr = ldr; a.ldm = ldm; a.relu = relu; a.out_f32 = out_f32 & 1; a.pool = pool;
  a.res_f32 = (dtype == 0 && (out_f32 & 2)) ? 1 : 0;
  a.res_pool = (out_f32 & 4) ? 1 : 0;
  if (a.res_pool && (!residual || (out_f32 & 2) || pool || KH != 1 || KW != 1 || pad != 0 || (long)Nimg * (a.Ho / 2) * (a.Wo / 2) * ldr * es >= (1L << 31) ||
                     (Cout & 7) || (ldy & 7) || (ldr & 7) || (relu_mask && (ldm & 7)))) return CDDMSL_ERR_ARG;
  if (a.res_f32 && ((Cout & 7) || (ldy & 7) || (ldr & 7))) return CDDMSL_ERR_ARG;
  long M = (long)Nimg * a.Ho * a.Wo;
  if (M > 0x7fffff00L) return CDDMSL_ERR_ARG;
  a.M = (int)M; a.cpp = Cin * es / 16; a.Kc = KH * KW * a.cpp;
  a.dWo = make_fastdiv((unsigned)a.Wo); a.dHo = make_fastdiv((unsigned)a.Ho);
  a.dcpp = make_fastdiv((unsigned)a.cpp); a.dKW = make_fastdiv((unsigned)KW);
  a.xrs = a.cpp; a.wrs = a.Kc; a.bx = a.bw = a.by = 0;
#ifdef CDDMSL_TILE_STAMPS
  a.tstamps = g_tile_stamps;
#endif
  if (a.M == 0) return CDDMSL_OK;
  a.nt_out = nt_out_for((long)a.M * Cout * 2);
  if (y8) {
    if (dtype != 0 || (out_f32 & 1) || ldy != Cout || !use_gemm256(a)) return CDDMSL_ERR_ARG;
    a.y8 = (char*)y8; a.q8 = q8; a.amax8 = (unsigned*)amax8;
  }
  return dtype == 0 ? conv_fwd_launch<__bf16>(a, (hipStream_t)stream) : conv_fwd_launch<float>(a, (hipStream_t)stream);
}

extern "C" int cddmsl_conv_fwd(const void* x, const void* w, void* y, const float* scale, const float* bias,
                               const void* residual, const void* relu_mask, int Nimg, int Hi, int Wi, int Cin,
                               int Cout, int KH, int KW, int stride, int pad, int pool, int ldy, int ldr, int ldm,
                               int relu, int out_f32, int dtype, void* stream) {
  return conv_fwd_impl(x, w, y, scale, bias, residual, relu_mask, Nimg, Hi, Wi, Cin, Cout, KH, KW, stride, pad, pool, ldy, ldr, ldm,
                       relu, out_f32, dtype, nullptr, nullptr, nullptr, stream);
}

extern "C" int cddmsl_conv_fwd_q8(const void* x, const void* w, void* y, const float* scale, const float* bias,
                                  const void* residual, const void* relu_mask, int Nimg, int Hi, int Wi, int Cin,
                                  int Cout, int KH, int KW, int stride, int pad, int relu, void* y8, const float* q8, float* amax8,
                                  void* stream) {
  if (!y8) return CDDMSL_ERR_ARG;
  return conv_fwd_impl(x, w, y, scale, bias, residual, relu_mask, Nimg, Hi, Wi, Cin, Cout, KH, KW, stride, pad, 0, Cout, Cout, Cout,
                       relu, 0, 0, y8, q8, amax8, stream);
}

extern "C" int cddmsl_conv_fwd_fp8(const void* x, const void* w, void* y, const float* scale, const float* bias,
                                   const void* residual, const void* relu_mask, int Nimg, int Hi, int Wi, int Cin, int Cout, int KH,
                                   int KW, int pad, int relu, int out_f32, void* y8, const float* q8, float* amax8, void* stream) {
  if (Nimg < 0 || Hi <= 0 || Wi <= 0 || Cin <= 0 || Cout <= 0 || KH <= 0 || KW <= 0 || (Cin % 128) != 0 || (out_f32 & ~1)) return CDDMSL_ERR_ARG;
  ConvArgs a;
  a.x = (const char*)x; a.w = (const char*)w; a.y = (char*)y; a.scale = scale; a.bias = bias;
  a.residual = (const char*)residual; a.relu_mask = (const char*)relu_mask;
  a.Nimg = Nimg; a.Hi = Hi; a.Wi = Wi; a.Cin = Cin; a.Cout = Cout; a.KH = KH; a.KW = KW; a.stride = 1; a.pad = pad;
  a.Ho = Hi + 2 * pad - KH + 1; a.Wo = Wi + 2 * pad - KW + 1;
  if (a.Ho <= 0 || a.Wo <= 0) return CDDMSL_ERR_ARG;
  a.ldy = a.ldr = a.ldm = Cout; a.relu = relu; a.out_f32 = out_f32; a.pool = 0; a.res_f32 = 0; a.res_pool = 0;
  long M = (long)Nimg * a.Ho * a.Wo;
  if (M > 0x7fffff00L) return CDDMSL_ERR_ARG;
  a.M = (int)M; a.cpp = Cin / 16; a.Kc = KH * KW * a.cpp;
  a.nt_out = nt_out_for(M * Cout * 2);
  a.dWo = make_fastdiv((unsigned)a.Wo); a.dHo = make_fastdiv((unsigned)a.Ho);
  a.dcpp = make_fastdiv((unsigned)a.cpp); a.dKW = make_fastdiv((unsigned)KW);
  a.xrs = a.cpp; a.wrs = a.Kc; a.bx = a.bw = a.by = 0;
  if (a.M == 0) return CDDMSL_OK;
  if (!gemm256_legal(a)) return CDDMSL_ERR_ARG;
  if (y8) {
    if (out_f32) return CDDMSL_ERR_ARG;
    a.y8 = (char*)y8; a.q8 = q8; a.amax8 = (unsigned*)amax8;
  }
  const long grid = (long)(a.Cout / 256) * ((a.M + 255) / 256);
  if (grid > 0x7fffffffL) return CDDMSL_ERR_ARG;
  g_last_kernel = 10;
  if (g_plan_only) return CDDMSL_OK;
  hipStream_t st = (hipStream_t)stream;
  if (KH == 1 && KW == 1 && pad == 0) launch256<fp8e4, false>(a, dim3((unsigned)grid, 1), st);
  else launch256<fp8e4, true>(a, dim3((unsigned)grid, 1), st);
  return launch_status();
}

static bool wgrad256_ok(const WgradArgs& a, int batch) {
  const char* e = getenv("CDDMSL_GEMM256");
  const int mode = e ? atoi(e) : 1;
  if (mode == 0) return false;
  if ((a.Cout & 255) || (a.K & 255) || (a.cpp & 7) || (a.ldd & 7)) return false;
  if (mode == 2) return true;
  const char* et = getenv("CDDMSL_WGRAD256_MIN");
  return (long)(a.Cout / 256) * (a.K / 256) * batch * ((a.M + WM - 1) / WM) >= (et ? atol(et) : 4000);
}
static bool wgrad256_span_ok(const WgradArgs& a) {
  const long rowb = (long)(a.ldd * 2 > a.xrs * 16 ? a.ldd * 2 : a.xrs * 16);
  return ((long)a.mtiles_per_split * WM + WM + 2L * a.Wi + 2) * rowb + (1L << 20) < (1L << 31);
}

template <int WAVES, int FR>
__global__ __launch_bounds__(256) void k_wgrad_reduce(const f32x4* ws, float* dw, const float* scale, int ntn, int ntk, int splits, int Cout, int K, int ldo) {
  constexpr int SLOTS = WAVES * FR * 64;
  constexpr int TN = WAVES == 8 ? 256 : 128;
  const int tile = blockIdx.x / (SLOTS / 256), q = (blockIdx.x % (SLOTS / 256)) * 256 + threadIdx.x;
  const int tile_k = tile % ntk, tile_n = tile / ntk;
  const long ntiles = (long)ntn * ntk;
  const f32x4* src = ws + (long)tile * SLOTS + q;
  f32x4 sum = {0.f, 0.f, 0.f, 0.f};
  int s = 0;
  for (; s + 4 <= splits; s += 4) {
    const f32x4 a = src[(s + 0) * ntiles * SLOTS], b = src[(s + 1) * ntiles * SLOTS], c = src[(s + 2) * ntiles * SLOTS], d = src[(s + 3) * ntiles * SLOTS];
    sum += (a + b) + (c + d);
  }
  for (; s < splits; ++s) sum += src[s * ntiles * SLOTS];
  const int wv = q / (FR * 64), j = (q / 64) % FR, lane = q & 63, r = lane & 31, h = lane >> 5, g4 = j & 3;
  int a, b, wn, wk;
  if (WAVES == 8) { a = j >> 3; b = (j >> 2) & 1; wn = wv >> 2; wk = wv & 3; }
  else { a = j >> 3; b = (j >> 2) & 1; wn = wv >> 1; wk = wv & 1; }
  const int n = tile_n * TN + wn * (WAVES == 8 ? 128 : 64) + a * 32 + 8 * g4 + 4 * h;
  const int k = tile_k * TN + wk * 64 + b * 32 + r;
  if (k >= K) return;
#pragma unroll
  for (int e = 0; e < 4; ++e)
    if (n + e < Cout) dw[(long)(n + e) * ldo + k] += sum[e] * (scale ? scale[n + e] : 1.f);
}

extern "C" int cddmsl_set_workspace(void* ptr, long bytes) {
  if (bytes < 0 || (ptr == nullptr && bytes != 0) || ((size_t)ptr & 15)) return CDDMSL_ERR_ARG;
  g_ws = ptr; g_ws_bytes = bytes;
  return CDDMSL_OK;
}
static bool use_workspace(long blocks, long tile_floats) {
  const char* e = getenv("CDDMSL_WGRAD_WS");
  if (e && atoi(e) == 0) return false;
  return g_ws != nullptr && blocks * tile_floats * 4 <= g_ws_bytes;
}

extern "C" int cddmsl_conv_wgrad(const void* x, const void* dy, float* dw, const float* scale, int Nimg, int Hi,
                                 int Wi, int Cin, int Cout, int KH, int KW, int stride, int pad, int pool, int ldd,
                                 int dtype, void* stream) {
  int es = dtype == 0 ? 2 : 4;
  if (dtype != 0 && dtype != 1) return CDDMSL_ERR_ARG;
  if (Nimg < 0 || Hi <= 0 || Wi <= 0 || Cin <= 0 || Cout <= 0 || KH <= 0 || KW <= 0 || stride <= 0) return CDDMSL_ERR_ARG;
  if ((Cin * es) % 16 != 0 || (Cout * es) % 16 != 0 || (ldd * es) % 16 != 0) return CDDMSL_ERR_ARG;
  if (pool && (KH != 1 || KW != 1 || pad != 0 || stride != 1)) return CDDMSL_ERR_ARG;
  WgradArgs a;
  a.x = (const char*)x; a.dy = (const char*)dy; a.dw = dw; a.scale = scale;
  a.Nimg = Nimg; a.Hi = Hi; a.Wi = Wi; a.Cin = Cin; a.Cout = Cout; a.KH = KH; a.KW = KW; a.stride = stride; a.pad = pad;
  a.ldd = ldd; a.pool = pool;
  if (pool) { a.Ho = Hi / 2; a.Wo = Wi / 2; }
  else { a.Ho = (Hi + 2 * pad - KH) / stride + 1; a.Wo = (Wi + 2 * pad - KW) / stride + 1; }
  if (a.Ho <= 0 || a.Wo <= 0) return CDDMSL_ERR_ARG;
  long M = (long)Nimg * a.Ho * a.Wo;
  if (M > 0x7fffff00L) return CDDMSL_ERR_ARG;
  a.M = (int)M; a.cpp = Cin * es / 16; a.Kc = KH * KW * a.cpp; a.K = KH * KW * Cin; a.ncc = Cout * es / 16;
  a.dWo = make_fastdiv((unsigned)a.Wo); a.dHo = make_fastdiv((unsigned)a.Ho);
  a.xrs = a.cpp; a.ldo = a.K; a.direct = 0; a.bx = a.bd = a.bo = 0;
#ifdef CDDMSL_TILE_STAMPS
  a.tstamps = g_tile_stamps;
#endif
  if (a.M == 0) return CDDMSL_OK;
  int cols = 256 / es;
  long tiles = (long)((Cout + cols - 1) / cols) * ((a.K + cols - 1) / cols);
  int total_mt = (a.M + WM - 1) / WM;
  const char* eb = getenv("CDDMSL_WGRAD_BLOCKS");
  const long target = eb ? atol(eb) : ((KH == 1 && KW == 1) ? 512 : 1024);
  long maxs = (total_mt + 7) / 8;
  long splits = 1;
  {
    const long r0 = (target + 511) / 512;
    double best = -1.0;
    for (long r = r0; r <= r0 + 1; ++r) {
      long c = (512 * r) / tiles;
      if (c < 1) c = 1;
      if (c > maxs) c = maxs;
      const int mps = (int)((total_mt + c - 1) / c);
      const long real = (total_mt + mps - 1) / mps, blocks = tiles * real, rounds = (blocks + 511) / 512;
      const double eff = (double)blocks / (512.0 * rounds);
      if (eff > best + 0.03) { best = eff; splits = c; }
      if (c == maxs) break;
    }
    if (eb) { splits = (target + tiles - 1) / tiles; if (splits > maxs) splits = maxs; }
  }
  if (splits < 1) splits = 1;
  a.mtiles_per_split = (int)((total_mt + splits - 1) / splits);
  splits = (total_mt + a.mtiles_per_split - 1) / a.mtiles_per_split;
  long grid = tiles * splits;
  if (grid > 0x7fffffffL) return CDDMSL_ERR_ARG;
  const bool same = !pool && stride == 1 && a.Ho == Hi && a.Wo == Wi;
  if (same && dtype == 0 && wgrad256_ok(a, 1)) {
    long tiles2 = (long)(Cout / 256) * (a.K / 256);
    long maxs2 = (total_mt + 15) / 16;
    long sp = 1;
    double best = -1.0;
    const char* eb2 = getenv("CDDMSL_WGRAD256_BLOCKS");
    for (int r = 1; r <= 6 && !eb2; ++r) {
      long c = (256L * r) / tiles2;
      if (c < 1) continue;
      if (c > maxs2) c = maxs2;
      const long blocks = tiles2 * c, rounds = (blocks + 255) / 256;
      const double eff = (double)blocks / (256.0 * rounds);
      if (eff > best + 0.02) { best = eff; sp = c; }
      if (c == maxs2) break;
    }
    if (eb2) { sp = (atol(eb2) + tiles2 - 1) / tiles2; if (sp > maxs2) sp = maxs2; }
    if (sp < 1) sp = 1;
    int keep = a.mtiles_per_split;
    a.mtiles_per_split = (int)((total_mt + sp - 1) / sp);
    sp = (total_mt + a.mtiles_per_split - 1) / a.mtiles_per_split;
    if (wgrad256_span_ok(a)) {
      g_last_kernel = 6;
      if (g_plan_only) return CDDMSL_OK;
      if (sp > 1 && use_workspace(tiles2 * sp, 65536)) {
        a.ws = (float*)g_ws;
        hipLaunchKernelGGL(k_wgrad256, dim3((unsigned)(tiles2 * sp)), dim3(512), 0, (hipStream_t)stream, a);
        hipLaunchKernelGGL((k_wgrad_reduce<8, 32>), dim3((unsigned)(tiles2 * 64)), dim3(256), 0, (hipStream_t)stream, (const f32x4*)g_ws, dw, scale,
                           Cout / 256, a.K / 256, (int)sp, Cout, a.K, a.ldo);
        return launch_status();
      }
      hipLaunchKernelGGL(k_wgrad256, dim3((unsigned)(tiles2 * sp)), dim3(512), 0, (hipStream_t)stream, a);
      return launch_status();
    }
    a.mtiles_per_split = keep;
  }
  g_last_kernel = same ? 5 : 4;
  if (g_plan_only) return CDDMSL_OK;
  if (same && dtype == 0 && splits > 1 && use_workspace(grid, 16384)) {
    a.ws = (float*)g_ws;
    hipLaunchKernelGGL(k_conv_wgrad_dma<__bf16>, dim3((unsigned)grid), dim3(256), 0, (hipStream_t)stream, a);
    hipLaunchKernelGGL((k_wgrad_reduce<4, 16>), dim3((unsigned)(tiles * 16)), dim3(256), 0, (hipStream_t)stream, (const f32x4*)g_ws, dw, scale,
                       (Cout + 127) / 128, (a.K + 127) / 128, (int)splits, Cout, a.K, a.ldo);
  } else if (same) {
    if (dtype == 0) hipLaunchKernelGGL(k_conv_wgrad_dma<__bf16>, dim3((unsigned)grid), dim3(256), 0, (hipStream_t)stream, a);
    else hipLaunchKernelGGL(k_conv_wgrad_dma<float>, dim3((unsigned)grid), dim3(256), 0, (hipStream_t)stream, a);
  } else {
    if (dtype == 0) hipLaunchKernelGGL(k_conv_wgrad<__bf16>, dim3((unsigned)grid), dim3(256), 0, (hipStream_t)stream, a);
    else hipLaunchKernelGGL(k_conv_wgrad<float>, dim3((unsigned)grid), dim3(256), 0, (hipStream_t)stream, a);
  }
  return launch_status();
}

extern "C" int cddmsl_conv_wgrad_fp8_ok(int Cin, int Cout, int KH, int KW, int pad, int ldd) {
  return (Cin % 256 == 0 && Cout % 256 == 0 && KH == KW && (KH & 1) && 2 * pad == KH - 1 && ldd % 16 == 0) ? 1 : 0;
}
extern "C" int cddmsl_conv_wgrad_fp8(const void* x8, const void* dy8, float* dw, const float* scale, int Nimg, int Hi, int Wi, int Cin,
                                     int Cout, int KH, int KW, int pad, int ldd, void* stream) {
  if (Nimg < 0 || Hi <= 0 || Wi <= 0 || !cddmsl_conv_wgrad_fp8_ok(Cin, Cout, KH, KW, pad, ldd) || ldd < Cout) return CDDMSL_ERR_ARG;
  WgradArgs a;
  a.x = (const char*)x8; a.dy = (const char*)dy8; a.dw = dw; a.scale = scale;
  a.Nimg = Nimg; a.Hi = Hi; a.Wi = Wi; a.Cin = Cin; a.Cout = Cout; a.KH = KH; a.KW = KW; a.stride = 1; a.pad = pad;
  a.ldd = ldd; a.pool = 0; a.Ho = Hi; a.Wo = Wi;
  const long M = (long)Nimg * Hi * Wi;
  if (M > 0x7fffff00L) return CDDMSL_ERR_ARG;
  a.M = (int)M; a.cpp = Cin / 16; a.Kc = KH * KW * a.cpp; a.K = KH * KW * Cin; a.ncc = Cout / 16;
  a.dWo = make_fastdiv((unsigned)a.Wo); a.dHo = make_fastdiv((unsigned)a.Ho);
  a.xrs = a.cpp; a.ldo = a.K; a.direct = 0; a.bx = a.bd = a.bo = 0;
  if (a.M == 0) return CDDMSL_OK;
  const int total_mt = (a.M + WM - 1) / WM;
  const long tiles = (long)(Cout / 256) * (a.K / 256), maxs = (total_mt + 15) / 16;
  long sp = 1;
  double best = -1.0;
  for (int r = 1; r <= 6; ++r) {
    long c = (256L * r) / tiles;
    if (c < 1) continue;
    if (c > maxs) c = maxs;
    const long blocks = tiles * c, rounds = (blocks + 255) / 256;
    const double eff = (double)blocks / (256.0 * rounds);
    if (eff > best + 0.02) { best = eff; sp = c; }
    if (c == maxs) break;
  }
  a.mtiles_per_split = (int)((total_mt + sp - 1) / sp);
  sp = (total_mt + a.mtiles_per_split - 1) / a.mtiles_per_split;
  const long rowb = ldd > a.xrs * 16 ? ldd : a.xrs * 16;
  if (((long)a.mtiles_per_split * WM + WM + 2L * Wi + 2) * rowb + (1L << 20) >= (1L << 31)) return CDDMSL_ERR_ARG;
  g_last_kernel = 12;
  if (g_plan_only) return CDDMSL_OK;
  if (sp > 1 && use_workspace(tiles * sp, 65536)) {
    a.ws = (float*)g_ws;
    hipLaunchKernelGGL(k_wgrad256_f8, dim3((unsigned)(tiles * sp)), dim3(512), 0, (hipStream_t)stream, a);
    hipLaunchKernelGGL((k_wgrad_reduce<8, 32>), dim3((unsigned)(tiles * 64)), dim3(256), 0, (hipStream_t)stream, (const f32x4*)g_ws, dw, scale,
                       Cout / 256, a.K / 256, (int)sp, Cout, a.K, a.ldo);
    return launch_status();
  }
  hipLaunchKernelGGL(k_wgrad256_f8, dim3((unsigned)(tiles * sp)), dim3(512), 0, (hipStream_t)stream, a);
  return launch_status();
}

extern "C" int cddmsl_gemm_nt_batched(const void* a, const void* w, void* c, const float* bias, int M, int N, int K, int lda,
                                      int ldb, int ldc, int batch, long sa, long sw, long sc, int out_f32, int dtype, void* stream) {
  int es = dtype == 0 ? 2 : 4;
  if (dtype != 0 && dtype != 1) return CDDMSL_ERR_ARG;
  if (M < 0 || N <= 0 || K <= 0 || batch < 0 || batch > 65535) return CDDMSL_ERR_ARG;
  if ((K * es) % 16 || (lda * es) % 16 || (ldb * es) % 16 || (sa * es) % 16 || (sw * es) % 16) return CDDMSL_ERR_ARG;
  if (M == 0 || batch == 0) return CDDMSL_OK;
  ConvArgs p;
  p.x = (const char*)a; p.w = (const char*)w; p.y = (char*)c; p.scale = nullptr; p.bias = bias; p.residual = nullptr; p.relu_mask = nullptr;
  p.Nimg = 1; p.Hi = 1; p.Wi = M; p.Cin = K; p.Ho = 1; p.Wo = M; p.Cout = N; p.KH = 1; p.KW = 1; p.stride = 1; p.pad = 0;
  p.ldy = ldc; p.ldr = 0; p.ldm = 0; p.relu = 0; p.out_f32 = out_f32; p.pool = 0; p.res_f32 = 0; p.res_pool = 0;
  p.M = M; p.cpp = K * es / 16; p.Kc = p.cpp;
  p.dWo = make_fastdiv((unsigned)M); p.dHo = make_fastdiv(1u); p.dcpp = make_fastdiv((unsigned)p.cpp); p.dKW = make_fastdiv(1u);
  p.xrs = lda * es / 16; p.wrs = ldb * es / 16;
  p.bx = sa * es; p.bw = sw * es; p.by = sc * (out_f32 ? 4 : es);
  g_batch = batch;
  int st = dtype == 0 ? conv_fwd_launch<__bf16>(p, (hipStream_t)stream) : conv_fwd_launch<float>(p, (hipStream_t)stream);
  g_batch = 1;
  return st;
}

extern "C" int cddmsl_gemm_tn_batched(const void* a, const void* b, void* out, int M, int N, int K, int lda, int ldb, int ldo,
                                      int batch, long sa, long sb, long so, int mode, int dtype, void* stream) {
  int es = dtype == 0 ? 2 : 4;
  if (dtype != 0 && dtype != 1) return CDDMSL_ERR_ARG;
  if (M <= 0 || N <= 0 || K <= 0 || batch <= 0 || batch > 65535 || mode < 0 || mode > 2) return CDDMSL_ERR_ARG;
  if ((K * es) % 16 || (N * es) % 16 || (lda * es) % 16 || (ldb * es) % 16 || (sa * es) % 16 || (sb * es) % 16) return CDDMSL_ERR_ARG;
  WgradArgs p;
  p.x = (const char*)b; p.dy = (const char*)a; p.dw = (float*)out; p.scale = nullptr;
  p.Nimg = 1; p.Hi = 1; p.Wi = M; p.Cin = K; p.Ho = 1; p.Wo = M; p.Cout = N; p.KH = 1; p.KW = 1; p.stride = 1; p.pad = 0;
  p.ldd = lda; p.pool = 0; p.M = M; p.cpp = K * es / 16; p.Kc = p.cpp; p.K = K; p.ncc = N * es / 16;
  p.dWo = make_fastdiv((unsigned)M); p.dHo = make_fastdiv(1u);
  p.xrs = ldb * es / 16; p.ldo = ldo; p.direct = mode;
  p.bx = sb * es; p.bd = sa * es; p.bo = so * (mode == 2 ? es : 4);
  int cols = 256 / es;
  long tiles = (long)((N + cols - 1) / cols) * ((K + cols - 1) / cols);
  int total_mt = (M + WM - 1) / WM;
  long splits = 1;
  if (mode == 0) {
    long want = (2048 + tiles * batch - 1) / (tiles * batch);
    long maxs = (total_mt + 7) / 8;
    splits = want < 1 ? 1 : (want > maxs ? maxs : want);
    if (splits < 1) splits = 1;
  }
  if (dtype == 0 && total_mt == 1 && N <= 64 && batch >= 64 && K % 128 == 0 && N % 8 == 0) {
    const long kt = K / 128;
    long bpb = (kt * batch + 4095) / 4096;
    if (bpb < 8) bpb = 8;
    if (bpb > batch) bpb = batch;
    const unsigned gy = (unsigned)((batch + bpb - 1) / bpb);
    g_last_kernel = 9;
    if (g_plan_only) return CDDMSL_OK;
#define CDDMSL_TNS(NG)                                                                                                               \
  case NG:                                                                                                                           \
    if (mode == 0) hipLaunchKernelGGL((k_gemm_tn_small<NG, 0>), dim3((unsigned)kt, gy), dim3(256), 0, (hipStream_t)stream, p, batch, (int)bpb);      \
    else if (mode == 1) hipLaunchKernelGGL((k_gemm_tn_small<NG, 1>), dim3((unsigned)kt, gy), dim3(256), 0, (hipStream_t)stream, p, batch, (int)bpb); \
    else hipLaunchKernelGGL((k_gemm_tn_small<NG, 2>), dim3((unsigned)kt, gy), dim3(256), 0, (hipStream_t)stream, p, batch, (int)bpb);                \
    break;
    switch (N / 8) { CDDMSL_TNS(1) CDDMSL_TNS(2) CDDMSL_TNS(3) CDDMSL_TNS(4) CDDMSL_TNS(5) CDDMSL_TNS(6) CDDMSL_TNS(7) CDDMSL_TNS(8) }
#undef CDDMSL_TNS
    return launch_status();
  }
  if (total_mt <= 4 && batch >= 64) {
    long bpb = (tiles * batch + 4095) / 4096, minb = (8 + total_mt - 1) / total_mt;
    if (bpb < minb) bpb = minb;
    if (bpb > batch) bpb = batch;
    const unsigned gy = (unsigned)((batch + bpb - 1) / bpb);
    g_last_kernel = 7;
    if (g_plan_only) return CDDMSL_OK;
    if (dtype == 0) hipLaunchKernelGGL(k_gemm_tn_stream<__bf16>, dim3((unsigned)tiles, gy), dim3(256), 0, (hipStream_t)stream, p, batch, (int)bpb);
    else hipLaunchKernelGGL(k_gemm_tn_stream<float>, dim3((unsigned)tiles, gy), dim3(256), 0, (hipStream_t)stream, p, batch, (int)bpb);
    return launch_status();
  }
  p.mtiles_per_split = (int)((total_mt + splits - 1) / splits);
  splits = (total_mt + p.mtiles_per_split - 1) / p.mtiles_per_split;
  long grid = tiles * splits;
  if (grid > 0x7fffffffL) return CDDMSL_ERR_ARG;
  g_last_kernel = 5;
  if (g_plan_only) return CDDMSL_OK;
  if (dtype == 0) hipLaunchKernelGGL(k_conv_wgrad_dma<__bf16>, dim3((unsigned)grid, (unsigned)batch), dim3(256), 0, (hipStream_t)stream, p);
  else hipLaunchKernelGGL(k_conv_wgrad_dma<float>, dim3((unsigned)grid, (unsigned)batch), dim3(256), 0, (hipStream_t)stream, p);
  return launch_status();
}

extern "C" int cddmsl_attnpool_dx(const void* pds, const void* zu, const float* g0, const unsigned long long* mbits, void* dx, float* gpos,
                                  int K, int H2, int P, int TP, int C, int dtype, void* stream) {
// ... 40 lines not shown
```

cddmsl_amd/hip.py:

```python
import ctypes
import os
from ctypes import c_float, c_int, c_long, c_void_p

import torch

from ._lib import check, lib, ptr, require_cuda, stream_ptr

DT = {torch.bfloat16: 0, torch.float32: 1}

_sigs_done = False


def _L():
    global _sigs_done
    L = lib()
    if not _sigs_done:
        vp, ci, cf = c_void_p, c_int, c_float
        L.cddmsl_last_kernel.argtypes = []
        L.cddmsl_plan_only.argtypes = [ci]
        L.cddmsl_conv_fwd.argtypes = [vp] * 7 + [ci] * 16 + [vp]
        L.cddmsl_conv_wgrad.argtypes = [vp] * 4 + [ci] * 12 + [vp]
        L.cddmsl_set_workspace.argtypes = [vp, c_long]
        L.cddmsl_weight_prep.argtypes = [vp] * 4 + [ci] * 5 + [vp]
        L.cddmsl_weight_prep_multi.argtypes = [vp, ci, ci, vp]
        L.cddmsl_preprocess.argtypes = [vp, vp] + [ci] * 6 + [vp, vp, ci, ci, vp]
        L.cddmsl_maxpool3s2_fwd.argtypes = [vp, vp] + [ci] * 5 + [vp]
        L.cddmsl_upsample_zero2.argtypes = [vp] * 4 + [ci] * 5 + [vp]
        L.cddmsl_meanpool_fwd.argtypes = [vp, vp, c_long, ci, ci, ci, vp]
        L.cddmsl_meanpool_bwd.argtypes = [vp, vp, c_long, ci, ci, ci, vp]
        L.cddmsl_preprocess224.argtypes = [vp, vp] + [ci] * 11 + [vp, vp, ci, vp]
        L.cddmsl_preprocess_batch.argtypes = [vp, vp, vp, ci, vp, ci, ci, ci, vp, vp, ci, ci, vp]
        L.cddmsl_preprocess224_batch.argtypes = [vp, vp, vp, ci, vp] + [ci] * 8 + [vp, vp, ci, vp]
        L.cddmsl_avgpool2_fwd.argtypes = [vp, vp] + [ci] * 5 + [vp]
        L.cddmsl_avgpool2_bwd.argtypes = [vp] * 4 + [ci] * 5 + [vp]
        L.cddmsl_avgpool2_bwd_q8.argtypes = [vp] * 4 + [ci] * 4 + [vp] * 4
        L.cddmsl_attn_tokens_fwd.argtypes = [vp] * 3 + [ci] * 5 + [vp]
        L.cddmsl_attn_tokens_bwd.argtypes = [vp] * 4 + [ci] * 5 + [vp]
        L.cddmsl_attnpool_softmax_fwd.argtypes = [vp] * 3 + [c_long, ci, ci, ci, cf, ci, vp]
        L.cddmsl_attnpool_softmax_bwd.argtypes = [vp] * 4 + [c_long, ci, ci, ci, cf, ci, vp]
        L.cddmsl_gemm_nt_batched.argtypes = [vp] * 4 + [ci] * 7 + [c_long] * 3 + [ci, ci, vp]
        L.cddmsl_gemm_tn_batched.argtypes = [vp] * 3 + [ci] * 7 + [c_long] * 3 + [ci, ci, vp]
        L.cddmsl_relu_bwd.argtypes = [vp, vp, vp, c_long, ci, ci, vp]
        L.cddmsl_colsum.argtypes = [vp, vp, c_long, ci, ci, ci, vp]
        L.cddmsl_sgd_clip_step.argtypes = [vp] * 4 + [ci, vp] + [cf] * 4 + [ci, vp]
        L.cddmsl_roi_align_forward.argtypes = [vp] * 5 + [ci] * 7 + [cf, ci, ci, ci, vp]
        L.cddmsl_roi_align_backward.argtypes = [vp] * 7 + [ci] * 7 + [cf, ci, ci, ci, vp]
        L.cddmsl_nms_anyorder.argtypes = [vp] * 4 + [ci, cf, vp, vp, vp]
        L.cddmsl_roi_align_nchw_anyorder.argtypes = [vp] * 3 + [ci] * 7 + [cf, ci, ci, ci, vp, vp, vp]
        L.cddmsl_roi_align_backward_nchw_anyorder.argtypes = [vp] * 3 + [ci] * 7 + [cf, ci, ci, ci, vp, vp, vp]
        L.cddmsl_quantize_fp8.argtypes = [vp] * 4 + [c_long, ci, vp]
        L.cddmsl_conv_fwd_fp8.argtypes = [vp] * 7 + [ci] * 10 + [vp] * 4
        L.cddmsl_conv_wgrad_fp8_ok.argtypes = [ci] * 6
        L.cddmsl_conv_wgrad_fp8.argtypes = [vp] * 4 + [ci] * 9 + [vp]
        L.cddmsl_conv_fwd_q8.argtypes = [vp] * 7 + [ci] * 10 + [vp] * 4
        L.cddmsl_fp8_dot_nt.argtypes = [vp] * 4 + [ci] * 4 + [vp]
        L.cddmsl_roi_align_forward_affine.argtypes = [vp] * 6 + [ci] * 8 + [cf, ci, ci, ci] + [vp] * 4
        L.cddmsl_roi_align_backward_pooled.argtypes = [vp] * 7 + [ci] * 7 + [cf, ci, ci, ci, vp]
        L.cddmsl_anchors.argtypes = [vp, vp, ci, ci, ci, cf, cf, vp]
        L.cddmsl_sort_desc.argtypes = [vp] * 5 + [ci, ci, vp, vp, vp]
        L.cddmsl_rpn_decode.argtypes = [vp] * 6 + [ci] * 5 + [cf] * 8 + [vp]
        L.cddmsl_nms.argtypes = [vp] * 5 + [ci, ci, cf, ci, vp]
        L.cddmsl_iou_match.argtypes = [vp, ci, vp, ci, vp, vp, vp, ci, cf, cf, ci, ci, ci, ci, vp]
        L.cddmsl_iou_match_batched.argtypes = [vp] * 7 + [ci] * 5 + [cf, cf] + [ci] * 4 + [vp]
        L.cddmsl_l2norm_fwd.argtypes = [vp, vp, vp, c_long, ci, cf, vp]
        L.cddmsl_l2norm_bwd.argtypes = [vp, vp, vp, vp, c_long, ci, vp]
        L.cddmsl_cosine_logits_fwd.argtypes = [vp] * 4 + [c_long, ci, ci, cf, cf, vp]
        L.cddmsl_cosine_logits_bwd.argtypes = [vp] * 5 + [c_long, ci, ci, cf, ci, vp]
        L.cddmsl_layernorm_fwd.argtypes = [vp] * 6 + [c_long, ci, cf, ci, vp]
        L.cddmsl_layernorm_bwd.argtypes = [vp] * 6 + [c_long, ci, ci, ci, vp]
        L.cddmsl_focal_ce_fwd.argtypes = [vp] * 4 + [c_long, ci, cf, ci, cf, vp]
        L.cddmsl_focal_ce_bwd.argtypes = [vp] * 5 + [c_long, ci, cf, ci, cf, vp]
        L.cddmsl_attn_small_fwd.argtypes = [vp] * 4 + [ci] * 8 + [cf, ci, vp]
        L.cddmsl_attn_small_bwd.argtypes = [vp] * 7 + [ci] * 8 + [cf, ci, vp]
        L.cddmsl_attn_tokens_fwd_mask.argtypes = [vp] * 4 + [ci] * 5 + [vp]
        L.cddmsl_attnpool_dx.argtypes = [vp] * 6 + [ci] * 6 + [vp]
        L.cddmsl_rpn_losses.argtypes = [vp, vp, vp, ci, vp, ci, vp, vp, vp, vp, c_long, cf, cf, cf, cf, cf, vp, vp, vp, vp, vp]
        L.cddmsl_box_l1.argtypes = [vp, ci, vp, ci, vp, vp, vp, cf, cf, cf, cf, cf, vp, vp, vp, vp]
        L.cddmsl_attn_last_fwd.argtypes = [vp] * 4 + [ci] * 8 + [cf, ci, vp]
        L.cddmsl_attn_last_bwd.argtypes = [vp] * 6 + [ci] * 8 + [cf, ci, vp]
        L.cddmsl_contrastive_fwd.argtypes = [vp] * 4 + [ci, ci, vp]
        L.cddmsl_contrastive_bwd.argtypes = [vp] * 5 + [ci, ci, vp]
        L.cddmsl_instance_boxes.argtypes = [vp] + [ci] * 4 + [vp, ci, vp, vp, vp, vp]
        L.cddmsl_text_embed.argtypes = [vp] * 4 + [c_long, ci, ci, ci, ci, vp]
        L.cddmsl_attn_causal_fwd.argtypes = [vp, vp] + [ci] * 6 + [cf, ci, vp]
        L.cddmsl_quick_gelu.argtypes = [vp, c_long, ci, vp]
        L.cddmsl_text_pool.argtypes = [vp] * 5 + [c_long, ci, ci, ci, cf, ci, vp]
        L.cddmsl_skinny_gemm_workspace.argtypes = [ci] * 3
        L.cddmsl_skinny_gemm.argtypes = [vp] * 6 + [c_long] + [ci] * 4 + [vp]
        L.cddmsl_lm_head_workspace.argtypes = [ci, ci]
        L.cddmsl_lm_head_argmax.argtypes = [vp, vp, vp, ci, vp, vp, c_long, ci, ci, ci, vp]
        L.cddmsl_decode_attn.argtypes = [vp] * 4 + [ci] * 6 + [cf, ci, vp]
        L.cddmsl_pos_embed.argtypes = [vp, ci] + [vp] * 4 + [c_long] + [ci] * 6 + [vp]
        L.cddmsl_gelu_new.argtypes = [vp, c_long, ci, vp]
        _sigs_done = True
    return L


class _Profiler:

    def __init__(self):
        self.on = False
        self.only = None
        self.events = []
        self.shapes = []

    def enable(self, only=None):
        self.on, self.only, self.events, self.shapes = True, (set(only) if only else None), [], []

    def begin(self, name=None, plan=None):
        if not self.on:
            return None
        if self.only is not None:
            if name is None and plan is not None:
                L = _L()
                L.cddmsl_plan_only(1)
                try:
                    plan()
                finally:
                    L.cddmsl_plan_only(0)
                name = _CONV_KERNEL.get(L.cddmsl_last_kernel())
            if name not in self.only:
                return None
        e = torch.cuda.Event(enable_timing=True)
        e.record()
        return e

    def end(self, e0, name, flops=0.0, shape=None, nbytes=0.0):
        if e0 is None:
            return
        e1 = torch.cuda.Event(enable_timing=True)
        e1.record()
        self.events.append((name, flops, e0, e1, nbytes))
        if shape is not None:
            self.shapes.append((name, shape, flops, e0, e1, nbytes))

    def by_shape(self):
        torch.cuda.synchronize()
        out = {}
        for name, shape, flops, e0, e1, nbytes in self.shapes:
            d = out.setdefault((name, shape), [0, 0.0, 0.0, 0.0])
            d[0] += 1
            d[1] += e0.elapsed_time(e1)
            d[2] += flops
            d[3] += nbytes
        return out

    def collect(self):
        torch.cuda.synchronize()
        out = {}
        for name, flops, e0, e1, nbytes in self.events:
            d = out.setdefault(name, {"flops": 0.0, "ms": 0.0, "launches": 0, "bytes": 0.0})
            d["flops"] += flops
            d["bytes"] += nbytes
            d["ms"] += e0.elapsed_time(e1)
            d["launches"] += 1
        self.on, self.only, self.events = False, None, []
        return out


PROFILE = _Profiler()
_CONV_KERNEL = {10: "k_conv_fwd256_fp8", 11: "k_conv_fwd2", 1: "k_conv_fwd", 2: "k_conv_fwd_reg", 3: "k_conv_fwd256", 4: "k_conv_wgrad", 5: "k_conv_wgrad_dma", 6: "k_wgrad256", 7: "k_gemm_tn_stream", 8: "k_conv3x3_small", 9: "k_gemm_tn_small", 12: "k_wgrad256_fp8"}


def _timed(name):
    def deco(fn):
        def wrapper(*a, **k):
            e0 = PROFILE.begin(name)
            r = fn(*a, **k)
            PROFILE.end(e0, name)
            return r
        wrapper.__name__, wrapper.__doc__ = fn.__name__, fn.__doc__
# ... 1091 lines not shown
```

include/cddmsl_hip.h:

```cpp
#ifndef CDDMSL_HIP_H
#define CDDMSL_HIP_H
#include <stddef.h>

#ifdef __cplusplus
extern "C" {
#endif

int cddmsl_abi_version(void);

int cddmsl_conv_fwd(const void* x, const void* w, void* y, const float* scale, const float* bias, const void* residual,
                    const void* relu_mask, int Nimg, int Hi, int Wi, int Cin, int Cout, int KH, int KW, int stride, int pad,
                    int pool, int ldy, int ldr, int ldm, int relu, int out_f32, int dtype, void* stream);
int cddmsl_set_workspace(void* ptr, long bytes);
int cddmsl_conv_wgrad(const void* x, const void* dy, float* dw, const float* scale, int Nimg, int Hi, int Wi, int Cin,
                      int Cout, int KH, int KW, int stride, int pad, int pool, int ldd, int dtype, void* stream);
int cddmsl_gemm_nt_batched(const void* a, const void* w, void* c, const float* bias, int M, int N, int K, int lda, int ldb, int ldc,
                           int batch, long sa, long sw, long sc, int out_f32, int dtype, void* stream);
int cddmsl_gemm_tn_batched(const void* a, const void* b, void* out, int M, int N, int K, int lda, int ldb, int ldo, int batch, long sa,
                           long sb, long so, int mode, int dtype, void* stream);
int cddmsl_last_kernel(void);
int cddmsl_plan_only(int on);
int cddmsl_weight_prep(const float* w, const float* scale, void* w_fwd, void* w_dgrad, int Cout, int KH, int KW, int Cin,
                       int dtype, void* stream);
int cddmsl_weight_prep_multi(const long long* table, int count, int dtype, void* stream);

int cddmsl_quantize_fp8(const void* x, void* y, const float* scale, float* amax, long numel, int src_dtype, void* stream);
int cddmsl_conv_fwd_fp8(const void* x, const void* w, void* y, const float* scale, const float* bias, const void* residual,
                        const void* relu_mask, int Nimg, int Hi, int Wi, int Cin, int Cout, int KH, int KW, int pad, int relu,
                        int out_f32, void* y8, const float* q8, float* amax8, void* stream);
int cddmsl_conv_fwd_q8(const void* x, const void* w, void* y, const float* scale, const float* bias, const void* residual,
                       const void* relu_mask, int Nimg, int Hi, int Wi, int Cin, int Cout, int KH, int KW, int stride, int pad,
                       int relu, void* y8, const float* q8, float* amax8, void* stream);
int cddmsl_fp8_dot_nt(const void* a, const void* b, float* c, const float* alpha, int R, int N, int K, int ldc, void* stream);
int cddmsl_conv_wgrad_fp8_ok(int Cin, int Cout, int KH, int KW, int pad, int ldd);
int cddmsl_conv_wgrad_fp8(const void* x8, const void* dy8, float* dw, const float* scale, int Nimg, int Hi, int Wi, int Cin, int Cout,
                          int KH, int KW, int pad, int ldd, void* stream);

int cddmsl_roi_align_forward(const void* x, const float* rois, void* y, void* y_pooled, int* dbg_grid, int N, int C, int H, int W,
                             int K, int ph, int pw, float spatial_scale, int sampling_ratio, int aligned, int dtype, void* stream);
int cddmsl_roi_align_backward(const void* dy, const float* rois, const int* roi_start, void* dx, float* ws_ay, float* ws_ax,
                              int* ws_fp, int N, int C, int H, int W, int K, int ph, int pw, float spatial_scale,
                              int sampling_ratio, int aligned, int dtype, void* stream);
int cddmsl_roi_align_forward_affine(const void* x, const float* rois, void* y, void* y_pooled, const float* scale,
                                    const float* bias, int relu, int N, int C, int H, int W, int K, int ph, int pw,
                                    float spatial_scale, int sampling_ratio, int aligned, int dtype, void* y8, const float* q8,
                                    float* amax8, void* stream);
int cddmsl_roi_align_backward_pooled(const void* dy, const float* rois, const int* roi_start, void* dx, float* ws_ay,
                                     float* ws_ax, int* ws_fp, int N, int C, int H, int W, int K, int ph, int pw,
                                     float spatial_scale, int sampling_ratio, int aligned, int dtype, void* stream);
int cddmsl_roi_align_nchw_anyorder(const void* input, const float* rois, void* output, int N, int C, int H, int W, int K, int ph, int pw,
                                   float spatial_scale, int sampling_ratio, int aligned, int dtype, void* temp, size_t* temp_bytes,
                                   void* stream);
int cddmsl_roi_align_backward_nchw_anyorder(const void* grad, const float* rois, void* grad_input, int N, int C, int H, int W, int K,
                                            int ph, int pw, float spatial_scale, int sampling_ratio, int aligned, int dtype, void* temp,
                                            size_t* temp_bytes, void* stream);

int cddmsl_anchors(const float* cell, float* out, int Hf, int Wf, int A, float stride, float offset, void* stream);
int cddmsl_sort_desc(const float* keys_in, float* keys_out, int* idx_scratch, int* order_out, const int* offsets, int N,
                     int total, void* temp, size_t* temp_bytes, void* stream);
int cddmsl_rpn_decode(const int* order, const float* deltas, const float* cell, const int* img_hw, float* boxes,
                      unsigned char* valid, int N, int Hf, int Wf, int A, int topk, float stride, float offset, float wx,
                      float wy, float ww, float wh, float scale_clamp, float min_size, void* stream);
int cddmsl_nms(const float* boxes, const unsigned char* valid, unsigned long long* mask_ws, int* keep, int* nkeep, int N,
               int n, float thr, int max_keep, void* stream);
int cddmsl_nms_anyorder(const float* boxes, const float* scores, long* keep, int* nkeep, int K, float iou_threshold, void* temp,
                        size_t* temp_bytes, void* stream);
int cddmsl_iou_match(const float* gt, int G, const float* preds, int P, long* matches, signed char* labels,
                     unsigned int* best_ws, int nthr, float t0, float t1, int l0, int l1, int l2, int allow_low_quality,
                     void* stream);

int cddmsl_iou_match_batched(const float* gt, const int* gt_off, const float* preds, const int* pred_off, long* matches,
                             signed char* labels, unsigned int* best_ws, int N, int P, int maxG, int totalG, int nthr, float t0,
                             float t1, int l0, int l1, int l2, int allow_low_quality, void* stream);

int cddmsl_attn_tokens_fwd(const void* x, const float* pos, void* tok, int K, int P, int TP, int C, int dtype, void* stream);
int cddmsl_attn_tokens_fwd_mask(const void* x, const float* pos, void* tok, unsigned long long* mbits, int K, int P, int TP, int C,
                                int dtype, void* stream);
int cddmsl_attnpool_dx(const void* pds, const void* zu, const float* g0, const unsigned long long* mbits, void* dx, float* gpos, int K,
                       int H2, int P, int TP, int C, int dtype, void* stream);
int cddmsl_attn_tokens_bwd(const void* dtok, const void* relu_mask, void* dx, float* gpos, int K, int P, int TP, int C, int dtype,
                           void* stream);
int cddmsl_attnpool_softmax_fwd(const float* S, float* p, void* pT, long K, int H, int P1, int TP, float scale, int dtype, void* stream);
int cddmsl_attnpool_softmax_bwd(const float* p, const float* dP, void* dsT, void* pds, long K, int H, int P1, int TP, float scale,
                                int dtype, void* stream);

int cddmsl_attn_small_fwd(const void* q, const void* k, const void* v, void* o, int nseq, int t, int heads, int dh, int ldq,
                          int ldk, int ldv, int ldo, float scale, int dtype, void* stream);
int cddmsl_attn_small_bwd(const void* q, const void* k, const void* v, const void* dout, void* dq, void* dk, void* dv, int nseq,
                          int t, int heads, int dh, int ldq, int ldk, int ldv, int ldo, float scale, int dtype, void* stream);
int cddmsl_attn_last_fwd(const void* q, const void* kv, void* o, float* p, int n, int t, int heads, int dh, int ldq, int ldkv, int voff,
                         int ldo, float scale, int dtype, void* stream);
int cddmsl_attn_last_bwd(const void* q, const void* kv, const void* dout, const float* p, void* dq, void* dkv, int n, int t, int heads,
                         int dh, int ldq, int ldkv, int voff, int ldo, float scale, int dtype, void* stream);

int cddmsl_text_embed(const long* ids, const void* tok, const float* pos, float* x, long rows, int t, int W, int vocab, int dtype,
                      void* stream);
int cddmsl_attn_causal_fwd(const void* qkv, void* o, int nseq, int t, int heads, int dh, int ldqkv, int ldo, float scale, int dtype,
                           void* stream);
int cddmsl_quick_gelu(void* x, long numel, int dtype, void* stream);
int cddmsl_text_pool(const float* x, const long* rows, const float* gamma, const float* beta, void* y, long R, int nout, int group,
                     int W, float eps, int dtype, void* stream);

int cddmsl_skinny_gemm_workspace(int M, int N, int K);
int cddmsl_skinny_gemm(const void* x, const void* w, const float* bias, const float* residual, void* y, float* ws, long ws_bytes, int M,
                       int N, int K, int epi, void* stream);
int cddmsl_lm_head_workspace(int M, int V);
int cddmsl_lm_head_argmax(const void* h, const void* wte, long* ids, int ld_ids, float* logits, void* ws, long ws_bytes, int M, int V,
                          int K, void* stream);
int cddmsl_decode_attn(const void* qkv, void* kc, void* vc, void* o, int nseq, int heads, int dh, int L, int Lmax, int ldqkv, float scale,
                       int dtype, void* stream);
int cddmsl_pos_embed(const long* ids, int ld_ids, const void* tab, const float* src, const float* wpe, float* x, long rows, int t, int pos0,
                     int W, int vocab, int npos, int dtype, void* stream);
int cddmsl_gelu_new(void* x, long numel, int dtype, void* stream);

int cddmsl_l2norm_fwd(const float* x, float* y, float* inv, long R, int D, float eps, void* stream);
int cddmsl_l2norm_bwd(const float* dy, const float* y, const float* inv, float* dx, long R, int D, void* stream);
int cddmsl_cosine_logits_fwd(const float* x, const float* wn, float* scores, float* inv, long R, int D, int Kc,
                             float temperature, float eps, void* stream);
int cddmsl_cosine_logits_bwd(const float* ds, const float* x, const float* wn, const float* inv, float* dx, long R, int D,
                             int Kc, float temperature, int accumulate, void* stream);
int cddmsl_layernorm_fwd(const float* x, const float* gamma, const float* beta, void* y, float* mean, float* rstd, long R, int D,
                         float eps, int dtype, void* stream);
int cddmsl_layernorm_bwd(const void* dy, const float* x, const float* gamma, const float* mean, const float* rstd, float* dx,
                         long R, int D, int accumulate, int dtype, void* stream);
int cddmsl_focal_ce_fwd(const float* logits, const long* target, float* row_loss, float* probs, long R, int C, float gamma,
                        int bg_class, float bg_weight, void* stream);
int cddmsl_focal_ce_bwd(const float* logits, const long* target, const float* probs, const float* gscale, float* dlogits, long R,
                        int C, float gamma, int bg_class, float bg_weight, void* stream);
int cddmsl_contrastive_fwd(const float* S, float* rlse, float* clse, float* loss, int n, int ld, void* stream);
int cddmsl_contrastive_bwd(const float* S, const float* rlse, const float* clse, const float* gloss, float* dS, int n, int ld,
                           void* stream);
int cddmsl_rpn_losses(const float* logits, const float* deltas, const long* pos, int npos, const long* neg, int nneg, const long* midx,
                      const float* gt, const long* gt_off, const float* anchors, long A, float wx, float wy, float ww, float wh, float inv_norm,
                      float* out2, const float* gout2, float* dlogits, float* ddeltas, void* stream);
int cddmsl_box_l1(const float* deltas, int ld, const long* fg, int nfg, const long* cls, const float* src, const float* tgt, float wx, float wy,
                  float ww, float wh, float inv_norm, float* out1, const float* gout1, float* ddeltas, void* stream);

int cddmsl_preprocess(const unsigned char* img, void* out, int n, int h, int w, int Hp, int Wp, int Cp, const float* mean3,
                      const float* std3, int div255, int dtype, void* stream);
int cddmsl_preprocess224(const unsigned char* img, void* out, int n, int h, int w, int Hp, int Wp, int RH, int RW, int top,
                         int left, int S, int Cp, const float* mean3, const float* std3, int dtype, void* stream);
int cddmsl_preprocess_batch(const unsigned char* const* imgs, const int* hs, const int* ws, int N, void* out, int Hp, int Wp, int Cp,
                            const float* mean3, const float* std3, int div255, int dtype, void* stream);
int cddmsl_preprocess224_batch(const unsigned char* const* imgs, const int* hs, const int* ws, int N, void* out, int Hp, int Wp, int RH,
                               int RW, int top, int left, int S, int Cp, const float* mean3, const float* std3, int dtype, void* stream);
int cddmsl_avgpool2_fwd(const void* x, void* y, int N, int H, int W, int C, int dtype, void* stream);
int cddmsl_avgpool2_bwd(const void* dy, const void* mask, const void* add, void* dx, int N, int H, int W, int C, int dtype,
                        void* stream);
int cddmsl_avgpool2_bwd_q8(const void* dy, const void* mask, const void* add, void* dx, int N, int H, int W, int C, void* y8,
                           const float* q8, float* amax8, void* stream);
int cddmsl_maxpool3s2_fwd(const void* x, void* y, int N, int H, int W, int C, int dtype, void* stream);
int cddmsl_upsample_zero2(const void* t, const void* mask, const void* add, void* dx, int N, int H, int W, int C, int dtype,
                          void* stream);
int cddmsl_meanpool_fwd(const void* x, float* y, long K, int P, int C, int dtype, void* stream);
int cddmsl_meanpool_bwd(const float* dy, void* dx, long K, int P, int C, int dtype, void* stream);
int cddmsl_relu_bwd(const void* g, const void* y, void* dx, long numel, int g_f32, int dtype, void* stream);
int cddmsl_colsum(const void* x, float* out, long rows, int cols, int period, int dtype, void* stream);
int cddmsl_sgd_clip_step(float** params, const float** grads, float** moms, const long* sizes, int count, float* norm_ws,
                         float lr, float momentum, float wd, float clip, int first_step, void* stream);

int cddmsl_instance_boxes(const void* maps, int B, int H, int W, int dtype, int* records, int max_records, int* counts, void* ws,
                          size_t* ws_bytes, void* stream);

#ifdef __cplusplus
}
#endif
#endif
```

Baseline: 156.2.

## Add position-major tap-skipping conv forward and wgrad kernels for padded 3x3 convs

Adds a position-major variant of the 256-tile forward conv and wgrad kernels. Each tile covers one output position across a batch of images, so taps that fall entirely into padding are skipped rather than loaded and multiplied as zeros. The forward path is on by default when a cost heuristic estimates enough padding savings. The wgrad path runs only when CDDMSL_TAP_SKIP=2. The trade-off is more tiles with strided row access and smaller effective M per position, which can hurt locality.

```diff
diff --git a/cddmsl_amd/csrc/gemm_conv.hip b/cddmsl_amd/csrc/gemm_conv.hip
--- a/cddmsl_amd/csrc/gemm_conv.hip
+++ b/cddmsl_amd/csrc/gemm_conv.hip
@@ -643,6 +643,7 @@
   const float* g0 = nullptr;
   const unsigned long long* mbits = nullptr;
   float* gpos = nullptr;
+  int pm_splits = 0;
   float* ws = nullptr;
 #ifdef CDDMSL_TILE_STAMPS
   unsigned long long* tstamps = nullptr;
@@ -1277,6 +1278,7 @@
   }
 }
 
+template <bool PM>
 __global__ __launch_bounds__(512) void k_wgrad256(WgradArgs p) {
   __shared__ __attribute__((aligned(16))) u32x4 lds[2 * 2 * 2 * 64 * 16];
   const int t = threadIdx.x, lane = t & 63;
@@ -1293,9 +1295,21 @@
   const int tile_k = bid % ntk; bid /= ntk;
   const int tile_n = bid % ntn; bid /= ntn;
   const int n0 = tile_n * 256, k0 = tile_k * 256;
-  const int mt0 = bid * p.mtiles_per_split;
-  const int nmt = min(p.mtiles_per_split, (p.M + WM - 1) / WM - mt0);
   const bool taps = !(p.KH == 1 && p.KW == 1);
+  const int pmP = p.Ho * p.Wo;
+  int pm_oy0 = 0, pm_ox0 = 0, pm_ny = 1, pm_nx = 1, pm_t0 = 0, pm_nmt = 0;
+  int pm_sh = 0;
+  if (PM) {
+    const int tp = (k0 >> 3) / p.cpp, ky_ = tp / p.KW, kx_ = tp - ky_ * p.KW;
+    pm_oy0 = max(0, p.pad - ky_); pm_ox0 = max(0, p.pad - kx_);
+    pm_ny = max(0, min(p.Ho, p.Hi + p.pad - ky_) - pm_oy0); pm_nx = max(0, min(p.Wo, p.Wi + p.pad - kx_) - pm_ox0);
+    pm_sh = (ky_ - p.pad) * p.Wi + (kx_ - p.pad);
+    const int total = ((p.Nimg + WM - 1) / WM) * pm_ny * pm_nx, per = (total + p.pm_splits - 1) / p.pm_splits;
+    pm_t0 = bid * per;
+    pm_nmt = max(0, min(per, total - pm_t0));
+  }
+  const int mt0 = PM ? 0 : bid * p.mtiles_per_split;
+  const int nmt = PM ? pm_nmt : min(p.mtiles_per_split, (p.M + WM - 1) / WM - mt0);
 
   const int rb = t >> 4, cl = (t & 15) ^ fsw(rb);
   const int gd = (cl >> 3) * 16 + (cl & 7);
@@ -1308,7 +1322,21 @@
   for (int i = 0; i < 2; ++i) {
     vd[i] = (unsigned)((i * 32 + rb) * p.ldd * 2 + gd * 16);
     vx[i] = (unsigned)((((i * 32 + rb) + ky * p.Wi + kx) * p.xrs + coff) * 16);
-  }
+    if (PM) {
+      vd[i] = (unsigned)((i * 32 + rb) * pmP * p.ldd * 2 + gd * 16);
+      vx[i] = (unsigned)(((i * 32 + rb) * pmP * p.xrs + coff) * 16);
+    }
+  }
+  struct PmWalk { int c, y, x; };
+  PmWalk wkd[2], wkx[2];
+  if (PM) {
+    const int nvp = max(1, pm_ny * pm_nx), c0 = pm_t0 / nvp, q0 = pm_t0 - c0 * nvp, y0 = q0 / max(1, pm_nx);
+    wkd[0] = wkd[1] = wkx[0] = wkx[1] = PmWalk{c0, y0, q0 - y0 * pm_nx};
+  }
+  auto pm_adv = [&](PmWalk& w) { if (++w.x == pm_nx) { w.x = 0; if (++w.y == pm_ny) { w.y = 0; ++w.c; } } };
+  const char* const pm_dbase = p.dy + (long)n0 * 2;
+  const char* const pm_xbase = p.x + (long)pm_sh * p.xrs * 16;
+  const long pm_dchunk = (long)WM * pmP * p.ldd * 2, pm_xchunk = (long)WM * pmP * p.xrs * 16;
   const __amdgpu_buffer_rsrc_t rd = __builtin_amdgcn_make_buffer_rsrc((void*)(p.dy + ((long)mt0 * WM * p.ldd + n0) * 2), 0, 0x80000000u, 0x00020000);
   const __amdgpu_buffer_rsrc_t rx = __builtin_amdgcn_make_buffer_rsrc((void*)(p.x + ((long)mt0 * WM - p.pad * p.Wi - p.pad) * p.xrs * 16), 0, 0x80000000u, 0x00020000);
   const unsigned dstep = (unsigned)(WM * p.ldd * 2), xstep = (unsigned)(WM * p.xrs * 16);
@@ -1318,6 +1346,19 @@
   auto stageD = [&](auto H, int buf, int T) {
     constexpr int h = decltype(H)::value;
     char* dst = L + (buf << 16) + (h << 14) + wvu * 1024;
+    if (PM) {
+      PmWalk& w = wkd[h];
+      const __amdgpu_buffer_rsrc_t r = __builtin_amdgcn_make_buffer_rsrc((void*)(pm_dbase + w.c * pm_dchunk), 0, 0x80000000u, 0x00020000);
+      const int so = ((pm_oy0 + w.y) * p.Wo + pm_ox0 + w.x) * p.ldd * 2;
+#pragma unroll
+      for (int i = 0; i < 2; ++i) {
+        const unsigned inv = (w.c * WM + i * 32 + rb < p.Nimg) ? 0u : 0x80000000u;
+        __builtin_amdgcn_raw_ptr_buffer_load_lds(r, (__attribute__((address_space(3))) void*)(dst + i * 8192 - h * 128), 16,
+                                                 (int)(vd[i] | inv), so, h * 128, 0);
+      }
+      pm_adv(w);
+      return;
+    }
 #pragma unroll
     for (int i = 0; i < 2; ++i) {
       const unsigned inv = (mrow + T * WM + i * 32 < p.M) ? 0u : 0x80000000u;
@@ -1327,6 +1368,7 @@
   };
   unsigned xinv[2];
   auto validX = [&](int T) {
+    if (PM) return;
 #pragma unroll
     for (int i = 0; i < 2; ++i) {
       const int m = mrow + T * WM + i * 32;
@@ -1344,6 +1386,19 @@
   auto stageX = [&](auto J, int buf, int T) {
     constexpr int j = decltype(J)::value;
     char* dst = L + (buf << 16) + (1 << 15) + (j << 14) + wvu * 1024;
+    if (PM) {
+      PmWalk& w = wkx[j];
+      const __amdgpu_buffer_rsrc_t r = __builtin_amdgcn_make_buffer_rsrc((void*)(pm_xbase + w.c * pm_xchunk), 0, 0x80000000u, 0x00020000);
+      const int so = ((pm_oy0 + w.y) * p.Wo + pm_ox0 + w.x) * p.xrs * 16;
+#pragma unroll
+      for (int i = 0; i < 2; ++i) {
+        const unsigned inv = (w.c * WM + i * 32 + rb < p.Nimg) ? 0u : 0x80000000u;
+        __builtin_amdgcn_raw_ptr_buffer_load_lds(r, (__attribute__((address_space(3))) void*)(dst + i * 8192 - j * 64), 16,
+                                                 (int)(vx[i] | inv), so, j * 64, 0);
+      }
+      pm_adv(w);
+      return;
+    }
 #pragma unroll
     for (int i = 0; i < 2; ++i)
       __builtin_amdgcn_raw_ptr_buffer_load_lds(rx, (__attribute__((address_space(3))) void*)(dst + i * 8192 - j * 64), 16,
@@ -1868,6 +1923,7 @@
 
 static thread_local int g_last_kernel = 0;
 static thread_local int g_plan_only = 0;
+static thread_local int g_last_tap_skip = 0;
 static thread_local int g_batch = 1;
 static inline int g_batch_peek() { return g_batch; }
 
@@ -1877,7 +1933,7 @@
 
 template <typename T, bool RPOOL, int EPI, bool PRE = false>
 __device__ __forceinline__ void tile_epilogue(const ConvArgs& p, f32x16 (&acc)[4][2], float* ep, int wr, int wc, int lane, int m0, int n0,
-                                              const u32x4 (*pre)[4] = nullptr, const f32x4* sb = nullptr) {
+                                              const u32x4 (*pre)[4] = nullptr, const f32x4* sb = nullptr, int rsm = 1, long nrows = -1) {
   constexpr int ES = Mma<T>::ES;
   const int r32 = lane & 31, hh = lane >> 5;
   const int cg = lane & 7, rr = lane >> 3;
@@ -1893,7 +1949,7 @@
   const bool f32out = EPI < 0 && (ES == 4 || p.out_f32 != 0);
   const int eso = f32out ? 4 : 2;
   const float relu_floor = p.relu ? 0.f : -__builtin_inff();
-  const long rows = p.M - m0;
+  const long rows = nrows >= 0 ? nrows : (long)p.M - m0;
   auto mk = [&](const char* base, long ld, int es) {
     long bytes = rows * ld * es;
     if (bytes > 0x7fffffffL) bytes = 0x7fffffffL;
@@ -1911,11 +1967,12 @@
     const bool in = m < p.M && (oy >> 1) < hp && (ox >> 1) < wp;
     return in ? (unsigned)((((img * hp + (oy >> 1)) * wp + (ox >> 1)) * (unsigned)p.ldr + (unsigned)n) * ES) : 0x80000000u;
   };
-  const unsigned vy = (unsigned)(((wr * 128 + rr) * p.ldy + n) * eso);
-  const unsigned vr = (unsigned)(((wr * 128 + rr) * p.ldr + n) * esr), vm = (unsigned)(((wr * 128 + rr) * p.ldm + n) * ES);
+  const int ldy_ = p.ldy * rsm, ldr_ = p.ldr * rsm, ldm_ = p.ldm * rsm;
+  const unsigned vy = (unsigned)((wr * 128 + rr) * ldy_ * eso + n * eso);
+  const unsigned vr = (unsigned)((wr * 128 + rr) * ldr_ * esr + n * esr), vm = (unsigned)((wr * 128 + rr) * ldm_ * ES + n * ES);
   const bool emit8 = EPI < 0 && ES == 2 && p.y8 != nullptr;
   const __amdgpu_buffer_rsrc_t ry8 = mk(p.y8, p.ldy, 1);
-  const unsigned vy8 = (unsigned)((wr * 128 + rr) * p.ldy + n);
+  const unsigned vy8 = (unsigned)((wr * 128 + rr) * ldy_ + n);
   const float q8s = emit8 && p.q8 ? p.q8[0] : 1.f;
   unsigned am8 = 0u;
   constexpr int DEPTH = ES == 2 ? 2 : 1;
@@ -1930,8 +1987,8 @@
 #pragma unroll
       for (int q = 0; q < ES / 2; ++q) {
         if (RPOOL) rres_[i][q] = __builtin_amdgcn_raw_buffer_load_b128(rres, pooled_off(m0 + wr * 128 + a * 32 + rr + 8 * i), q * 16, 0);
-        else if (has_res && !rf32) rres_[i][q] = __builtin_amdgcn_raw_buffer_load_b128(rres, vr, (a * 32 + 8 * i) * p.ldr * ES + q * 16, CDDMSL_LOAD_AUX);
-        if (has_msk) rmsk_[i][q] = __builtin_amdgcn_raw_buffer_load_b128(rmsk, vm, (a * 32 + 8 * i) * p.ldm * ES + q * 16, CDDMSL_LOAD_AUX);
+        else if (has_res && !rf32) rres_[i][q] = __builtin_amdgcn_raw_buffer_load_b128(rres, vr, (a * 32 + 8 * i) * ldr_ * ES + q * 16, CDDMSL_LOAD_AUX);
+        if (has_msk) rmsk_[i][q] = __builtin_amdgcn_raw_buffer_load_b128(rmsk, vm, (a * 32 + 8 * i) * ldm_ * ES + q * 16, CDDMSL_LOAD_AUX);
       }
   };
   if (PRE && DEPTH == 2) {
@@ -1941,7 +1998,7 @@
       for (int i = 0; i < 4; ++i) {
         if (EPI & 1) {
           rresb[d % DEPTH][i][0] = pre[d][i];
-          if (EPI & 2) rmskb[d % DEPTH][i][0] = __builtin_amdgcn_raw_buffer_load_b128(rmsk, vm, (d * 32 + 8 * i) * p.ldm * ES, CDDMSL_LOAD_AUX);
+          if (EPI & 2) rmskb[d % DEPTH][i][0] = __builtin_amdgcn_raw_buffer_load_b128(rmsk, vm, (d * 32 + 8 * i) * ldm_ * ES, CDDMSL_LOAD_AUX);
         } else rmskb[d % DEPTH][i][0] = pre[d][i];
       }
   } else if (DEPTH == 2 && !rf32) { fetch(0, rresb[0], rmskb[0]); fetch(1, rresb[DEPTH - 1], rmskb[DEPTH - 1]); }
@@ -1959,7 +2016,7 @@
     if (rf32) {
 #pragma unroll
       for (int f = 0; f < 8; ++f)
-        rresb[(f >> 2) % DEPTH][f & 3][0] = __builtin_amdgcn_raw_buffer_load_b128(rres, vr, (a * 32 + 8 * (f >> 1)) * p.ldr * 4 + (f & 1) * 16, 0);
+        rresb[(f >> 2) % DEPTH][f & 3][0] = __builtin_amdgcn_raw_buffer_load_b128(rres, vr, (a * 32 + 8 * (f >> 1)) * ldr_ * 4 + (f & 1) * 16, 0);
     }
     u32x4 (*rres_)[ES / 2] = rresb[a % DEPTH];
     u32x4 (*rmsk_)[ES / 2] = rmskb[a % DEPTH];
@@ -2023,12 +2080,12 @@
 #pragma unroll
         for (int j = 0; j < 8; ++j) if (!(mv[j] > 0.f)) v[j] = 0.f;
       }
-      const unsigned so = (unsigned)((a * 32 + 8 * i) * p.ldy * eso);
+      const unsigned so = (unsigned)((a * 32 + 8 * i) * ldy_ * eso);
       if (emit8) {
 #pragma unroll
         for (int j = 0; j < 8; ++j) am8 = absmax_bits(am8, v[j]);
         const u32x2 o8 = {pack4_e4m3(v[0] * q8s, v[1] * q8s, v[2] * q8s, v[3] * q8s), pack4_e4m3(v[4] * q8s, v[5] * q8s, v[6] * q8s, v[7] * q8s)};
-        __builtin_amdgcn_raw_buffer_store_b64(o8, ry8, vy8, (unsigned)((a * 32 + 8 * i) * p.ldy), CDDMSL_STORE_AUX);
+        __builtin_amdgcn_raw_buffer_store_b64(o8, ry8, vy8, (unsigned)((a * 32 + 8 * i) * ldy_), CDDMSL_STORE_AUX);
         asm volatile("s_nop 4" ::: "memory");
         asm volatile("" :: "v"(o8));
       }
@@ -2060,8 +2117,9 @@
   }
 }
 
-template <typename T, bool TAPS, bool RPOOL = false, int EPI = -1, bool PERSIST = false, bool SPLITK = false>
+template <typename T, bool TAPS, bool RPOOL = false, int EPI = -1, bool PERSIST = false, bool SPLITK = false, bool PM = false>
 __global__ __launch_bounds__(512) void k_conv_fwd256(ConvArgs p) {
+  static_assert(!PM || (TAPS && !RPOOL && !PERSIST && !SPLITK), "position-major: one-tile grid of a filter with taps");
   __shared__ __attribute__((aligned(16))) u32x4 lds[2 * 2 * 2 * 128 * KCH];
   const int t_in = threadIdx.x;
   p.x += (long)blockIdx.y * p.bx; p.w += (long)blockIdx.y * p.bw; p.y += (long)blockIdx.y * p.by;
@@ -2081,9 +2139,10 @@
   const int wvu = __builtin_amdgcn_readfirstlane(t >> 6);
   const int wr = wvu >> 2, wc = wvu & 3;
   const int tile_n = lbid % ntn, tile_m = lbid / ntn;
-  const int m0 = tile_m * 256, n0 = tile_n * 256;
+  const int pmP = p.Ho * p.Wo;
+  const int pm_g = PM ? tile_m / pmP : 0, pm_q = PM ? tile_m - pm_g * pmP : 0;
+  const int m0 = PM ? pm_g * 256 * pmP + pm_q : tile_m * 256, n0 = tile_n * 256;
   const int cl = (t & 7) ^ ((t >> 4) & 7);
-  const int nkt = SPLITK ? min(p.kper, (p.Kc >> 3) - kt0) : (p.Kc >> 3);
   const int tpt = p.cpp >> 3;
 
   auto rowoff = [&](int m, int& iy0, int& ix0) {
@@ -2102,15 +2161,21 @@
   for (int h = 0; h < 2; ++h)
 #pragma unroll
     for (int i = 0; i < 2; ++i) {
+      vinv[h][i] = 0;
+      vb[h][i] = (unsigned)(((2 * i + (t >> 8)) * 64 + h * 32 + ((t >> 3) & 31)) * p.wrs + cl) * 16;
+      if (PM) {
+        const int r = i * 128 + h * 64 + (t >> 3);
+        va[h][i] = (unsigned)(r * pmP * p.xrs + cl) * 16;
+        if (pm_g * 256 + r >= p.Nimg) va[h][i] |= 0x80000000u;
+        continue;
+      }
       const int m = m0 + i * 128 + h * 64 + (t >> 3);
       const bool vm = m < p.M;
       const long ro = rowoff(vm ? m : m0, iy0[h][i], ix0[h][i]);
       va[h][i] = (unsigned)(ro - base_a) + cl * 16;
       if (!vm) { iy0[h][i] = -(1 << 20); if (!TAPS) va[h][i] |= 0x80000000u; }
-      vinv[h][i] = 0;
-      vb[h][i] = (unsigned)(((2 * i + (t >> 8)) * 64 + h * 32 + ((t >> 3) & 31)) * p.wrs + cl) * 16;
-    }
-  if (TAPS) {
+    }
+  if (TAPS && !PM) {
     unsigned xm[2][2] = {{0, 0}, {0, 0}};
     for (int kx = 0; kx < p.KW; ++kx)
 #pragma unroll
@@ -2128,6 +2193,22 @@
   const int step_row = ((p.Wi - (p.KW - 1)) * p.xrs - (p.cpp - KCH)) * 16;
   int left[2] = {tpt, tpt}, tap[2] = {0, 0}, kxs[2] = {0, 0};
   unsigned soa[2] = {0, 0}, sob[2] = {0, 0};
+  unsigned pm_valid = 0;
+  int leftb[2] = {tpt, tpt}, tapb[2] = {0, 0};
+  auto pm_next = [&](int tp) { return tp + 1 + (int)__builtin_ctz((pm_valid >> (tp + 1)) | 0x40000000u); };
+  auto pm_tapoff = [&](int tp) {
+    const int ky = (int)fdiv((unsigned)tp, p.dKW), kx = tp - ky * p.KW;
+    return (unsigned)((ky * p.Wi + kx) * p.xrs * 16);
+  };
+  if (PM) {
+    for (int ky = 0; ky < p.KH; ++ky)
+      for (int kx = 0; kx < p.KW; ++kx)
+        if ((unsigned)(iyb + ky) < (unsigned)p.Hi && (unsigned)(ixb + kx) < (unsigned)p.Wi) pm_valid |= 1u << (ky * p.KW + kx);
+    const int tap0 = (int)__builtin_ctz(pm_valid | 0x40000000u);
+#pragma unroll
+    for (int h = 0; h < 2; ++h) { tap[h] = tapb[h] = tap0; soa[h] = pm_tapoff(tap0); sob[h] = (unsigned)(tap0 * p.cpp * 16); }
+  }
+  const int nkt = PM ? tpt * __builtin_popcount(pm_valid) : SPLITK ? min(p.kper, (p.Kc >> 3) - kt0) : (p.Kc >> 3);
   if (SPLITK) {
     const int tap0 = TAPS ? kt0 / tpt : 0, within = TAPS ? kt0 - tap0 * tpt : kt0;
     const int ky0 = TAPS ? tap0 / p.KW : 0, kx0 = tap0 - ky0 * p.KW;
@@ -2146,10 +2227,13 @@
 #pragma unroll
     for (int i = 0; i < 2; ++i) {
       unsigned v = va[h][i];
-      if (TAPS) v |= __builtin_amdgcn_ubfe(vinv[h][i], (unsigned)tap[h], 1u) << 31;
+      if (TAPS && !PM) v |= __builtin_amdgcn_ubfe(vinv[h][i], (unsigned)tap[h], 1u) << 31;
       blds16(ra_rsrc, v, soa[h], dst + i * 8192);
     }
-    if (TAPS) {
+    if (PM) {
+      if (--left[h] == 0) { left[h] = tpt; tap[h] = pm_next(tap[h]); soa[h] = pm_tapoff(tap[h]); }
+      else soa[h] += KCH * 16;
+    } else if (TAPS) {
       int step = KCH * 16;
       if (--left[h] == 0) {
         left[h] = tpt; ++tap[h];
@@ -2163,7 +2247,8 @@
     char* dst = L + (buf << 16) + (1 << 15) + (j << 14) + wvu * 1024;
 #pragma unroll
     for (int i = 0; i < 2; ++i) blds16(rb_rsrc, vb[j][i], sob[j], dst + i * 8192);
-    sob[j] += KCH * 16;
+    if (PM && --leftb[j] == 0) { leftb[j] = tpt; tapb[j] = pm_next(tapb[j]); sob[j] = (unsigned)(tapb[j] * p.cpp * 16); }
+    else sob[j] += KCH * 16;
   };
   using I0 = std::integral_constant<int, 0>;
   using I1 = std::integral_constant<int, 1>;
@@ -2248,6 +2333,8 @@
 #endif
 
   constexpr bool PREF = EPI > 0 && !RPOOL && Mma<T>::ES == 2 && !SPLITK;
+  const int ep_rsm = PM ? pmP : 1;
+  const long ep_rows = PM ? (long)(min(256, p.Nimg - pm_g * 256) - 1) * pmP + 1 : (long)p.M - m0;
   u32x4 pre[2][4];
   f32x4 sb[4];
   auto ktile = [&](int kt, auto LAST) {
@@ -2275,10 +2362,10 @@
     } else if (PREF) {
       const bool is_res = (EPI & 1) != 0;
       const char* base = is_res ? p.residual : p.relu_mask;
-      const int ld = is_res ? p.ldr : p.ldm;
-      long bytes = ((long)p.M - m0) * ld * 2;
+      const int ld1 = is_res ? p.ldr : p.ldm, ld = ld1 * ep_rsm;
+      long bytes = ep_rows * ld1 * 2;
       if (bytes > 0x7fffffffL) bytes = 0x7fffffffL;
-      const __amdgpu_buffer_rsrc_t rs = __builtin_amdgcn_make_buffer_rsrc((void*)(base + (long)m0 * ld * 2), 0, (int)bytes, 0x00020000);
+      const __amdgpu_buffer_rsrc_t rs = __builtin_amdgcn_make_buffer_rsrc((void*)(base + (long)m0 * ld1 * 2), 0, (int)bytes, 0x00020000);
       const unsigned vo = (unsigned)(((wr * 128 + (lane >> 3)) * ld + n0 + wc * 64 + (lane & 7) * 8) * 2);
 #pragma unroll
       for (int a = 0; a < 2; ++a)
@@ -2330,7 +2417,7 @@
         }
     return;
   }
-  tile_epilogue<T, RPOOL, EPI, PREF>(p, acc, (float*)lds + wvu * 4096, wr, wc, lane, m0, n0, pre, sb);
+  tile_epilogue<T, RPOOL, EPI, PREF>(p, acc, (float*)lds + wvu * 4096, wr, wc, lane, m0, n0, pre, sb, ep_rsm, ep_rows);
 #ifdef CDDMSL_TILE_STAMPS
   if (p.tstamps && lane == 0) {
     if (!PERSIST) asm volatile("s_waitcnt vmcnt(0)" ::: "memory");
@@ -2649,10 +2736,48 @@
     default: hipLaunchKernelGGL((k_conv_fwd256<T, TAPS, false, 3>), grid, dim3(512), 0, st, a); break;
   }
 }
+
+static double tap_valid_share(int H, int KH, int pad) {
+  long v = 0;
+  for (int k = 0; k < KH; ++k) { const int d = k > pad ? k - pad : pad - k; if (H > d) v += H - d; }
+  return (double)v / ((double)KH * H);
+}
+static bool tap_skip_legal(const ConvArgs& a) {
+  if (a.pool || a.res_pool || a.out_f32 || a.res_f32 || a.y8 || g_batch_peek() != 1) return false;
+  if (a.stride != 1 || a.KH != a.KW || a.KH < 3 || !(a.KH & 1) || 2 * a.pad != a.KH - 1 || a.Ho != a.Hi || a.Wo != a.Wi) return false;
+  long rowb = (long)a.xrs * 16;
+  if ((long)a.ldy * 2 > rowb) rowb = (long)a.ldy * 2;
+  if (a.residual && (long)a.ldr * 2 > rowb) rowb = (long)a.ldr * 2;
+  if (a.relu_mask && (long)a.ldm * 2 > rowb) rowb = (long)a.ldm * 2;
+  const long P = (long)a.Ho * a.Wo;
+  if ((256L * P + 2L * a.Wi + 2) * rowb + (1L << 20) >= (1L << 31)) return false;
+  return (long)(a.Cout / 256) * ((a.Nimg + 255) / 256) * P <= 0x7fffffffL;
+}
+static bool use_tap_skip(const ConvArgs& a) {
+  const char* e = getenv("CDDMSL_TAP_SKIP");
+  const int mode = e ? atoi(e) : 1;
+  if (mode == 0 || !tap_skip_legal(a)) return false;
+  if (mode == 2) return true;
+  const double pm = (double)((a.Nimg + 255) / 256) * 256.0 * a.Ho * a.Wo * tap_valid_share(a.Hi, a.KH, a.pad) * tap_valid_share(a.Wi, a.KW, a.pad);
+  const double rm = (double)((a.M + 255) / 256) * 256.0;
+  return pm <= 0.85 * rm;
+}
+template <typename T> void launch256_tap_skip(const ConvArgs& a, hipStream_t st) {
+  if constexpr (std::is_same<T, __bf16>::value) {
+    const dim3 grid((unsigned)((a.Cout / 256) * ((a.Nimg + 255) / 256) * a.Ho * a.Wo), 1);
+    switch ((a.residual ? 1 : 0) | (a.relu_mask ? 2 : 0)) {
+      case 0: hipLaunchKernelGGL((k_conv_fwd256<T, true, false, 0, false, false, true>), grid, dim3(512), 0, st, a); break;
+      case 1: hipLaunchKernelGGL((k_conv_fwd256<T, true, false, 1, false, false, true>), grid, dim3(512), 0, st, a); break;
+      case 2: hipLaunchKernelGGL((k_conv_fwd256<T, true, false, 2, false, false, true>), grid, dim3(512), 0, st, a); break;
+      default: hipLaunchKernelGGL((k_conv_fwd256<T, true, false, 3, false, false, true>), grid, dim3(512), 0, st, a); break;
+    }
+  }
+}
 template <> void launch256<float, false>(const ConvArgs& a, dim3 grid, hipStream_t st) { hipLaunchKernelGGL((k_conv_fwd256<float, false, false, -1>), grid, dim3(512), 0, st, a); }
 template <> void launch256<float, true>(const ConvArgs& a, dim3 grid, hipStream_t st) { hipLaunchKernelGGL((k_conv_fwd256<float, true, false, -1>), grid, dim3(512), 0, st, a); }
 
 template <typename T> int conv_fwd_launch(ConvArgs& a, hipStream_t st) {
+  g_last_tap_skip = 0;
   int ntn = (a.Cout + BN - 1) / BN, ntm = (a.M + BM - 1) / BM;
   long grid = (long)ntn * ntm;
   if (grid <= 0) return CDDMSL_OK;
@@ -2688,9 +2813,12 @@
   if (use_gemm256(a)) {
     grid = (long)(a.Cout / 256) * ((a.M + 255) / 256);
     g_last_kernel = 3;
+    const bool pm = sizeof(T) == 2 && use_tap_skip(a);
+    g_last_tap_skip = pm ? 1 : 0;
     if (g_plan_only) return CDDMSL_OK;
     const dim3 g256((unsigned)grid, (unsigned)g_batch);
-    if (a.res_pool) hipLaunchKernelGGL((k_conv_fwd256<T, false, true>), g256, dim3(512), 0, st, a);
+    if (pm) launch256_tap_skip<T>(a, st);
+    else if (a.res_pool) hipLaunchKernelGGL((k_conv_fwd256<T, false, true>), g256, dim3(512), 0, st, a);
     else if (a.KH == 1 && a.KW == 1 && a.pad == 0) launch256<T, false>(a, g256, st);
     else launch256<T, true>(a, g256, st);
   } else if (a.pool) { g_last_kernel = 2; if (g_plan_only) return CDDMSL_OK; hipLaunchKernelGGL(k_conv_fwd_reg<T>, dim3((unsigned)grid), dim3(256), 0, st, a); }
@@ -2705,6 +2833,7 @@
 extern "C" void cddmsl_debug_tile_stamps(unsigned long long* p) { g_tile_stamps = p; }
 #endif
 extern "C" int cddmsl_last_kernel(void) { return g_last_kernel; }
+extern "C" int cddmsl_last_tap_skip(void) { return g_last_tap_skip; }
 extern "C" int cddmsl_plan_only(int on) { const int was = g_plan_only; g_plan_only = on; return was; }
 
 static int nt_out_for(long out_bytes) {
@@ -2813,6 +2942,14 @@
   const char* et = getenv("CDDMSL_WGRAD256_MIN");
   return (long)(a.Cout / 256) * (a.K / 256) * batch * ((a.M + WM - 1) / WM) >= (et ? atol(et) : 4000);
 }
+static bool wgrad_tap_skip(const WgradArgs& a) {
+  const char* e = getenv("CDDMSL_TAP_SKIP");
+  if (!e || atoi(e) != 2) return false;
+  if (a.pool || a.stride != 1 || a.KH != a.KW || a.KH < 3 || !(a.KH & 1) || 2 * a.pad != a.KH - 1 || a.Ho != a.Hi || a.Wo != a.Wi) return false;
+  if ((a.cpp & 31) || a.KH * a.KW > 31) return false;
+  const long rowb = (long)(a.ldd * 2 > a.xrs * 16 ? a.ldd * 2 : a.xrs * 16), P = (long)a.Ho * a.Wo;
+  return ((long)WM * P + P + 2L * a.Wi + 2) * rowb + (1L << 20) < (1L << 31);
+}
 static bool wgrad256_span_ok(const WgradArgs& a) {
   const long rowb = (long)(a.ldd * 2 > a.xrs * 16 ? a.ldd * 2 : a.xrs * 16);
   return ((long)a.mtiles_per_split * WM + WM + 2L * a.Wi + 2) * rowb + (1L << 20) < (1L << 31);
@@ -2879,6 +3016,7 @@
 #ifdef CDDMSL_TILE_STAMPS
   a.tstamps = g_tile_stamps;
 #endif
+  g_last_tap_skip = 0;
   if (a.M == 0) return CDDMSL_OK;
   int cols = 256 / es;
   long tiles = (long)((Cout + cols - 1) / cols) * ((a.K + cols - 1) / cols);
@@ -2928,17 +3066,47 @@
     int keep = a.mtiles_per_split;
     a.mtiles_per_split = (int)((total_mt + sp - 1) / sp);
     sp = (total_mt + a.mtiles_per_split - 1) / a.mtiles_per_split;
+    if (wgrad_tap_skip(a)) {
+      const int nch = (Nimg + WM - 1) / WM;
+      const long fewest = (long)nch * (Hi > pad ? Hi - pad : 0) * (Wi > pad ? Wi - pad : 0);
+      long maxs3 = fewest / 16 > 1 ? fewest / 16 : 1, sp3 = 1;
+      double best3 = -1.0;
+      for (int r = 1; r <= 6 && !eb2; ++r) {
+        long c = (256L * r) / tiles2;
+        if (c < 1) continue;
+        if (c > maxs3) c = maxs3;
+        const long blocks = tiles2 * c, rounds = (blocks + 255) / 256;
+        const double eff = (double)blocks / (256.0 * rounds);
+        if (eff > best3 + 0.02) { best3 = eff; sp3 = c; }
+        if (c == maxs3) break;
+      }
+      if (eb2) { sp3 = (atol(eb2) + tiles2 - 1) / tiles2; if (sp3 > maxs3) sp3 = maxs3; }
+      if (sp3 < 1) sp3 = 1;
+      a.pm_splits = (int)sp3;
+      g_last_kernel = 6;
+      g_last_tap_skip = 1;
+      if (g_plan_only) return CDDMSL_OK;
+      if (sp3 > 1 && use_workspace(tiles2 * sp3, 65536)) {
+        a.ws = (float*)g_ws;
+        hipLaunchKernelGGL(k_wgrad256<true>, dim3((unsigned)(tiles2 * sp3)), dim3(512), 0, (hipStream_t)stream, a);
+        hipLaunchKernelGGL((k_wgrad_reduce<8, 32>), dim3((unsigned)(tiles2 * 64)), dim3(256), 0, (hipStream_t)stream, (const f32x4*)g_ws, dw, scale,
+                           Cout / 256, a.K / 256, (int)sp3, Cout, a.K, a.ldo);
+        return launch_status();
+      }
+      hipLaunchKernelGGL(k_wgrad256<true>, dim3((unsigned)(tiles2 * sp3)), dim3(512), 0, (hipStream_t)stream, a);
+      return launch_status();
+    }
     if (wgrad256_span_ok(a)) {
       g_last_kernel = 6;
       if (g_plan_only) return CDDMSL_OK;
       if (sp > 1 && use_workspace(tiles2 * sp, 65536)) {
         a.ws = (float*)g_ws;
-        hipLaunchKernelGGL(k_wgrad256, dim3((unsigned)(tiles2 * sp)), dim3(512), 0, (hipStream_t)stream, a);
+        hipLaunchKernelGGL(k_wgrad256<false>, dim3((unsigned)(tiles2 * sp)), dim3(512), 0, (hipStream_t)stream, a);
         hipLaunchKernelGGL((k_wgrad_reduce<8, 32>), dim3((unsigned)(tiles2 * 64)), dim3(256), 0, (hipStream_t)stream, (const f32x4*)g_ws, dw, scale,
                            Cout / 256, a.K / 256, (int)sp, Cout, a.K, a.ldo);
         return launch_status();
       }
-      hipLaunchKernelGGL(k_wgrad256, dim3((unsigned)(tiles2 * sp)), dim3(512), 0, (hipStream_t)stream, a);
+      hipLaunchKernelGGL(k_wgrad256<false>, dim3((unsigned)(tiles2 * sp)), dim3(512), 0, (hipStream_t)stream, a);
       return launch_status();
     }
     a.mtiles_per_split = keep;
diff --git a/cddmsl_amd/hip.py b/cddmsl_amd/hip.py
--- a/cddmsl_amd/hip.py
+++ b/cddmsl_amd/hip.py
@@ -17,6 +17,7 @@
     if not _sigs_done:
         vp, ci, cf = c_void_p, c_int, c_float
         L.cddmsl_last_kernel.argtypes = []
+        L.cddmsl_last_tap_skip.argtypes = []
         L.cddmsl_plan_only.argtypes = [ci]
         L.cddmsl_conv_fwd.argtypes = [vp] * 7 + [ci] * 16 + [vp]
         L.cddmsl_conv_wgrad.argtypes = [vp] * 4 + [ci] * 12 + [vp]
diff --git a/include/cddmsl_hip.h b/include/cddmsl_hip.h
--- a/include/cddmsl_hip.h
+++ b/include/cddmsl_hip.h
@@ -19,6 +19,7 @@
 int cddmsl_gemm_tn_batched(const void* a, const void* b, void* out, int M, int N, int K, int lda, int ldb, int ldo, int batch, long sa,
                            long sb, long so, int mode, int dtype, void* stream);
 int cddmsl_last_kernel(void);
+int cddmsl_last_tap_skip(void);
 int cddmsl_plan_only(int on);
 int cddmsl_weight_prep(const float* w, const float* scale, void* w_fwd, void* w_dgrad, int Cout, int KH, int KW, int Cin,
                        int dtype, void* stream);
```

After: 133.5. 14.5% lower.
